# leoelm/Bayesian_inference_for_NN

Measured on AMD Instinct MI355X. Metric: posterior samples/sec (grad-steps/sec) on MLP 784->200->10, batch 1024, higher is better.
Workload: dtype f32; 1 GPU; SGLD, MLP 784->200->10 (D=159010), synthetic MNIST-shaped 48000x784 fp32 resident in HBM, batch 1024 (last batch of an epoch 896), 1 chain per GPU, device-resident run replayed from hipGraphs; seed=2024, parallelism=independent chains x1 (replicas only, no data-path collective)

## Files before the change

### bayesian_inference_for_nn_amd/_build.py

```python

from __future__ import annotations

import fcntl
import glob
import os
import shutil
import subprocess

CSRC = os.path.join(os.path.dirname(os.path.abspath(__file__)), "csrc")
LIB = os.path.join(CSRC, "libpyz.so")
SOURCES = ["pyz_api.hip"]


class NoCompiler(RuntimeError):
    """hipcc is not installed (as opposed to: hipcc ran and failed)."""


def _inputs():
    return ([os.path.join(CSRC, f) for f in SOURCES] + sorted(glob.glob(os.path.join(CSRC, "*.h"))) +
            [os.path.join(CSRC, "..", "..", "include", "pyz.h")])


def _stale() -> bool:
    if not os.path.exists(LIB):
        return True
    t = os.path.getmtime(LIB)
    return any(os.path.exists(p) and os.path.getmtime(p) > t for p in _inputs())


def build(force: bool = False, verbose: bool = False) -> str:
    if not force and not _stale():
        return LIB
    hipcc = shutil.which("hipcc") or "/opt/rocm/bin/hipcc"
    if not os.path.exists(hipcc):
        raise NoCompiler("hipcc not found: cannot build the gfx950 library")
    with open(os.path.join(CSRC, ".build.lock"), "w") as lock:
        fcntl.flock(lock, fcntl.LOCK_EX)
        try:
            if not force and not _stale():
                return LIB
            tmp = LIB + f".tmp{os.getpid()}"
            cmd = [hipcc, "-O3", "-std=c++17", "--offload-arch=gfx950", "-fPIC", "-shared", "-Wall",
                   "-Wno-unused-function", "-Wno-pass-failed"] + SOURCES + ["-o", tmp]
            if verbose:
                print(" ".join(cmd))
            res = subprocess.run(cmd, cwd=CSRC, capture_output=True, text=True)
            if res.returncode != 0:
                if os.path.exists(tmp):
                    os.remove(tmp)
                raise RuntimeError("hipcc failed:\n" + res.stdout + res.stderr)
            os.replace(tmp, LIB)
        finally:
            fcntl.flock(lock, fcntl.LOCK_UN)
    return LIB


if __name__ == "__main__":
    print(build(force=True, verbose=True))
```

### bayesian_inference_for_nn_amd/csrc/pyz_api.hip

```cpp

#include <algorithm>
#include <climits>
#include <cmath>
#include <cstring>
#include <vector>

#include "pyz_common.h"
#include "pyz_corrupt.h"
#include "pyz_fsvi.h"
#include "pyz_fused.h"
#include "pyz_gemm.h"
#include "pyz_gemm_ring.h"
#include "pyz_hmc_fused.h"
#include "pyz_hmc_multi.h"
#include "pyz_input_grad.h"
#include "pyz_pilco.h"
#include "pyz_kernels.h"
#include "pyz_predict_moments.h"
#include "pyz_surface.h"
#include "pyz_rng.h"
#include "pyz_sgld_chains.h"
#include "pyz_sgld_lanes.h"
#include "pyz_members.h"

// ... 4 lines not shown

void drop_graphs(pyz_mlp *m);

int ensure_bytes(void **ptr, size_t *cap, size_t need, pyz_mlp *m) {
  if (*cap >= need) return PYZ_OK;
  if (*ptr) {
    PYZ_HIP(hipDeviceSynchronize());
    PYZ_HIP(hipFree(*ptr));
    drop_graphs(m);
  }
  *ptr = nullptr;
  *cap = 0;
  PYZ_HIP(hipMalloc(ptr, need));
  m->ws_bytes += need;
  *cap = need;
  return PYZ_OK;
}

struct Extra {
  size_t grad_cap = 0, grad2_cap = 0, qsave_cap = 0, part_cap = 0, part2_cap = 0, scal_cap = 0;
  void *hm_buf = nullptr;
  size_t hm_cap = 0;
  void *hm_res_buf = nullptr;
  size_t hm_res_cap = 0;
  void *fwd_part = nullptr;
  size_t fwd_part_cap = 0;
  void *gs_res_buf = nullptr;
  size_t gs_res_cap = 0;
  PyzGraphCache<1> hm_graphs;
  double *part2 = nullptr;
  void *tab_host = nullptr;
  size_t tab_host_cap = 0;
  hipEvent_t tab_ev[2] = {};
  unsigned long long tab_count = 0;
  float2 *tab_bc = nullptr;
  int tab_bc_cap = 0;
  static constexpr int AR_GRAPHS = 32;
  PyzGraphCache<AR_GRAPHS> adam_graphs;
  static constexpr int UP_SLOTS = 64;
  unsigned char *up_host = nullptr;
  size_t up_slot_bytes = 0;
  hipEvent_t up_ev[UP_SLOTS] = {};
  unsigned long long up_count = 0;
  bool hm_fed = false;
  int hm_path = 0;
  unsigned long long hm_sig = 0;
  void *hr_buf = nullptr;
  float *hr_tab = nullptr;
  size_t hr_tab_cap = 0;
  unsigned char *hr_host = nullptr;
  size_t hr_host_cap = 0;
  hipEvent_t hr_ev[2] = {};
  unsigned long long hr_count = 0;
  PyzGraphCache<PYZ_GRAPH_CHUNKS> hmc_run_graphs;
  void *fsvi_buf = nullptr;
  size_t fsvi_cap = 0;
};

}

struct pyz_mlp_full : pyz_mlp {
  Extra x;
};

namespace {

inline pyz_mlp_full *full(pyz_mlp *m) { return static_cast<pyz_mlp_full *>(m); }

void drop_graphs(pyz_mlp *m) {
  m->graphs.drop();
  full(m)->x.hm_graphs.drop();
  full(m)->x.hmc_run_graphs.drop();
  full(m)->x.adam_graphs.drop();
}

int need_grad(pyz_mlp *m, int P) {
  m->grad_owner = 2;
  return ensure_bytes((void **)&m->grad, &full(m)->x.grad_cap, sizeof(float) * (size_t)P * m->D + 64, m);
}
int need_grad2(pyz_mlp *m, int P) {
  return ensure_bytes((void **)&m->grad2, &full(m)->x.grad2_cap, sizeof(float) * (size_t)P * m->D + 64, m);
}
int need_qsave(pyz_mlp *m, int P) {
  return ensure_bytes((void **)&m->qsave, &full(m)->x.qsave_cap, sizeof(float) * (size_t)P * m->D + 64, m);
}
int need_part(pyz_mlp *m, size_t n_doubles) {
  return ensure_bytes((void **)&m->part, &full(m)->x.part_cap, sizeof(double) * n_doubles, m);
}
int need_part2(pyz_mlp *m, size_t n_doubles, bool keep_kernel_matrix = false) {
  if (!keep_kernel_matrix) m->km_valid = false;
  return ensure_bytes((void **)&full(m)->x.part2, &full(m)->x.part2_cap, sizeof(double) * n_doubles, m);
}

int check_call(const pyz_mlp *m, int P, int batch) {
  if (!m) return pyz_fail(PYZ_E_INVALID, "null plan");
  if (batch <= 0 || batch > m->max_batch)
    return pyz_fail(PYZ_E_SHAPE, "batch %d outside [1, %d] of the plan", batch, m->max_batch);
  if (P <= 0 || P > m->max_p)
    return pyz_fail(PYZ_E_SHAPE, "particle count %d outside [1, %d] of the plan", P, m->max_p);
  return PYZ_OK;
}

inline bool aligned16(const void *p) { return (reinterpret_cast<uintptr_t>(p) & 15u) == 0; }

int set_ctl(pyz_mlp *m, int slot, int batch, float lr, long long n, long long row_off, int i, hipStream_t st,
            int slot0 = 0, int n_run = 0) {
  m->pend_on = false;
  PYZ_LAUNCH(k_set_ctl, dim3(1), dim3(1), 0, st, m->ctl + slot, batch, lr, n, row_off, i, slot0, n_run);
  PYZ_LAUNCH_CHECK();
  return PYZ_OK;
}

void set_ctl_lazy(pyz_mlp *m, int batch, float lr, long long n) {
  m->pend = StepCtl{};
  m->pend.batch = batch;
  m->pend.lr = lr;
  m->pend.n = n;
  m->pend_on = true;
}

void flush_ctl(pyz_mlp *m, hipStream_t st) {
  if (!m->pend_on) return;
  m->pend_on = false;
  PYZ_LAUNCH(k_set_ctl, dim3(1), dim3(1), 0, st, m->ctl, m->pend.batch, m->pend.lr, m->pend.n, m->pend.row_off, m->pend.i,
                     m->pend.slot0, 0);
}

DenseArgs forward_args(pyz_mlp *m, int l, const float *theta, long long theta_ps, const float *x, const int32_t *row_idx,
                       const StepCtl *ctl, float *gather_out) {
  DenseArgs g{};
  g.K = m->dims[l];
  g.N = m->dims[l + 1];
  if (l == 0) {
    g.in = x;
    g.in_pstride = 0;
    g.row_idx = row_idx;
    g.gather_out = row_idx ? gather_out : nullptr;
  } else {
    g.in = m->act[l - 1];
    g.in_pstride = (long long)m->max_batch * g.K;
    g.row_idx = nullptr;
  }
  g.lda = g.K;
  g.theta = theta;
  g.theta_pstride = theta_ps;
  g.w_off = m->w_off[l];
  g.out = m->act[l];
  g.out_pstride = (long long)m->max_batch * g.N;
  g.act = m->acts[l];
  g.vec = (g.K % 8 == 0) && aligned16(g.in) ? 1 : 0;
  g.ctl = ctl;
  if (l == 0 && m->pend_on && ctl == m->ctl) {
    g.init = m->pend;
    g.init_on = 1;
    m->pend_on = false;
  }
  return g;
}

void launch_forward(pyz_mlp *m, const float *theta, long long theta_ps, int P, const float *x,
                    const int32_t *row_idx, int grid_batch, const StepCtl *ctl, hipStream_t st,
                    float *gather_out = nullptr, int l_end = -1, const StepCtl *gate = nullptr, int gate_mod = 0) {
  if (l_end < 0) l_end = m->L;
  for (int l = 0; l < l_end; ++l) {
    DenseArgs g = forward_args(m, l, theta, theta_ps, x, row_idx, ctl, gather_out);
    g.wt = pyz_wt_for(P);
    g.gate = gate;
    g.gate_mod = gate_mod;
    if (pyz_launch_fwd_ring(g, grid_batch, P, st)) continue;
    if (!g.row_idx && !g.init_on && !g.gather_out) g.rows_cap = std::min(grid_batch, m->max_batch);
    pyz_launch_fwd(g, grid_batch, P, st);
  }
}

void launch_loss(pyz_mlp *m, int P, const void *y, const int32_t *row_idx, int grid_batch, const StepCtl *ctl,
                 bool want_delta, hipStream_t st) {
  LossArgs g{};
  const int C = m->dims[m->L];
  g.out_last = m->act[m->L - 1];
  g.pstride = (long long)m->max_batch * C;
  g.C = C;
  g.y = y;
  g.delta = want_delta ? m->delta[m->L - 1] : nullptr;
  g.part = m->part;
  g.nblk = cdiv(m->max_batch, 256);
  g.act_last = m->acts[m->L - 1];
  g.ctl = ctl;
  g.row_idx = row_idx;
  dim3 grid(cdiv(grid_batch, 256), P);
  if ((int)grid.x < g.nblk) g.nblk = grid.x;
  if (m->loss == PYZ_LOSS_SCCE)
    PYZ_LAUNCH(k_loss_scce, grid, dim3(256), 0, st, g);
  else
    PYZ_LAUNCH(k_loss_mse, grid, dim3(256), 0, st, g);
}

inline int loss_nblk(const pyz_mlp *m, int grid_batch) { return std::min(cdiv(m->max_batch, 256), cdiv(grid_batch, 256)); }

void launch_backward(pyz_mlp *m, const float *theta, long long theta_ps, int P, const float *x,
                     const int32_t *row_idx, int grid_batch, const StepCtl *ctl, float *grad, hipStream_t st,
                     float *grad_sq = nullptr) {
  for (int l = m->L - 1; l >= 0; --l) {
    const int K = m->dims[l], N = m->dims[l + 1];
    if (l > 0) {
      DenseArgs g{};
      g.K = K;
      g.N = N;
      g.in = m->delta[l];
      g.in_pstride = (long long)m->max_batch * N;
      g.lda = N;
      g.theta = theta;
      g.theta_pstride = theta_ps;
      g.w_off = m->w_off[l];
      g.out = m->delta[l - 1];
      g.out_pstride = (long long)m->max_batch * K;
      g.aux = m->act[l - 1];
      g.aux_pstride = (long long)m->max_batch * K;
      g.act = m->acts[l - 1];
      g.vec = (N % 8 == 0) && (m->w_off[l] % 4 == 0) && (P == 1 || theta_ps % 4 == 0) && aligned16(theta) ? 1 : 0;
      g.ctl = ctl;
      pyz_launch_bwd_data(g, grid_batch, P, st);
    }
    DenseArgs g{};
    g.K = K;
    g.N = N;
    if (l == 0) {
      g.in = x;
      g.in_pstride = 0;
      g.row_idx = row_idx;
    } else {
      g.in = m->act[l - 1];
      g.in_pstride = (long long)m->max_batch * K;
    }
    g.lda = K;
    g.aux = m->delta[l];
    g.aux_pstride = (long long)m->max_batch * N;
    g.out = grad;
    g.out_pstride = m->D;
    g.w_off = m->w_off[l];
    g.ctl = ctl;
    if (grad_sq) pyz_launch_bwd_weight_sq(g, grad_sq, grid_batch, st);
    else pyz_launch_bwd_weight(g, grid_batch, P, st);
  }
}

inline bool can_fuse(const pyz_mlp *m) { return m->dims[m->L] <= 32; }

void launch_head(pyz_mlp *m, const float *theta, long long theta_ps, int P, const float *x, const void *y,
                 const int32_t *row_idx, int grid_batch, const StepCtl *ctl, bool want_delta, hipStream_t st,
                 const StepCtl *gate = nullptr, int gate_mod = 0, int k_split = 0) {
  const int l = m->L - 1;
  HeadArgs g{};
  g.gate = gate;
  g.gate_mod = gate_mod;
  if (k_split > 1) {
    g.hparts = static_cast<const float *>(full(m)->x.fwd_part);
    g.n_hparts = k_split;
    g.hpart_stride = (long long)m->max_batch * m->dims[l];
    g.bias_prev = theta + m->w_off[l - 1] + (long long)m->dims[l - 1] * m->dims[l];
    g.h_store = m->act[l - 1];
  }
  g.K = m->dims[l];
  g.N = m->dims[l + 1];
  if (l == 0) {
    g.hin = x;
    g.hin_pstride = 0;
    g.gather_hin = 1;
  } else {
    g.hin = m->act[l - 1];
    g.hin_pstride = (long long)m->max_batch * g.K;
    g.gather_hin = 0;
  }
  g.lda = g.K;
  g.row_idx = row_idx;
  g.theta = theta;
  g.theta_pstride = theta_ps;
  g.w_off = m->w_off[l];
  g.loss = m->loss;
  g.act_last = m->acts[l];
  g.act_prev = l > 0 ? m->acts[l - 1] : PYZ_ACT_LINEAR;
  g.vec = (g.K % 8 == 0) && aligned16(g.hin) ? 1 : 0;
  g.y = y;
  g.out_last = m->act[l];
  g.delta_last = want_delta ? m->delta[l] : nullptr;
  g.delta_prev = (want_delta && l > 0) ? m->delta[l - 1] : nullptr;
  g.last_pstride = (long long)m->max_batch * g.N;
  g.prev_pstride = (long long)m->max_batch * g.K;
  g.part = m->part;
  g.ctl = ctl;
  g.wt = pyz_wt_for(P);
  if (m->pend_on && ctl == m->ctl) {
    g.init = m->pend;
    g.init_on = 1;
    m->pend_on = false;
  }
  static const int rows_on = pyz_env_int("PYZ_HEAD_ROWS", 1);
  const int UT = g.K <= 64 ? 1 : g.K <= 256 ? 4 : g.K <= 512 ? 8 : g.K <= 1024 ? 16 : 0;
  const int NP = g.N <= 4 ? 4 : g.N <= 8 ? 8 : g.N <= 12 ? 12 : g.N <= 16 ? 16 : g.N <= 24 ? 24 : 32;
  if (rows_on && UT && UT * NP <= 128) {
    g.nblk = grid_batch;
    m->cur_nblk = g.nblk;
    static const int rw_rows = pyz_env_int("PYZ_HEAD_RW_ROWS", 32768);
    const int RW = (long long)P * grid_batch >= rw_rows ? 4 : 1;
    const dim3 grid((unsigned)cdiv(cdiv(grid_batch, RW), 4), P), block(256);
    if (g.n_hparts > 0) {
      if (NP == 4) PYZ_LAUNCH((k_head_rows<4, 4, 1, true>), grid, block, 0, st, g);
      else if (NP == 8) PYZ_LAUNCH((k_head_rows<4, 8, 1, true>), grid, block, 0, st, g);
      else if (NP == 12) PYZ_LAUNCH((k_head_rows<4, 12, 1, true>), grid, block, 0, st, g);
      else PYZ_LAUNCH((k_head_rows<4, 16, 1, true>), grid, block, 0, st, g);
      return;
    }
#define PYZ_HEAD_ROWS_CASE(U, C)                                                               \
  if (UT == U && NP == C) {                                                                    \
    if (RW == 4) PYZ_LAUNCH((k_head_rows<U, C, 4>), grid, block, 0, st, g);                     \
    else PYZ_LAUNCH((k_head_rows<U, C, 1>), grid, block, 0, st, g);                            \
    return;                                                                                    \
  }
    PYZ_HEAD_ROWS_CASE(1, 4) PYZ_HEAD_ROWS_CASE(1, 8) PYZ_HEAD_ROWS_CASE(1, 12) PYZ_HEAD_ROWS_CASE(1, 16)
    PYZ_HEAD_ROWS_CASE(1, 24) PYZ_HEAD_ROWS_CASE(1, 32)
    PYZ_HEAD_ROWS_CASE(4, 4) PYZ_HEAD_ROWS_CASE(4, 8) PYZ_HEAD_ROWS_CASE(4, 12) PYZ_HEAD_ROWS_CASE(4, 16)
    PYZ_HEAD_ROWS_CASE(4, 24) PYZ_HEAD_ROWS_CASE(4, 32)
    PYZ_HEAD_ROWS_CASE(8, 4) PYZ_HEAD_ROWS_CASE(8, 8) PYZ_HEAD_ROWS_CASE(8, 12) PYZ_HEAD_ROWS_CASE(8, 16)
    PYZ_HEAD_ROWS_CASE(16, 4) PYZ_HEAD_ROWS_CASE(16, 8)
#undef PYZ_HEAD_ROWS_CASE
  }
  g.nblk = cdiv(grid_batch, 32);
  m->cur_nblk = g.nblk;
  static const int head_waves = pyz_env_int("PYZ_HEAD_WAVES", 8) >= 8 ? 8 : 4;
  PYZ_LAUNCH(k_head, dim3(g.nblk, P), dim3(64 * head_waves), head_waves * 4096 + 2 * 32 * 33 * 4 + 64, st, g);
}

void launch_bwd_data_hidden(pyz_mlp *m, const float *theta, long long theta_ps, int P, int grid_batch,
                            const StepCtl *ctl, hipStream_t st) {
  for (int l = m->L - 2; l >= 1; --l) {
    const int K = m->dims[l], N = m->dims[l + 1];
    DenseArgs g{};
    g.K = K;
    g.N = N;
    g.in = m->delta[l];
    g.in_pstride = (long long)m->max_batch * N;
    g.lda = N;
    g.theta = theta;
    g.theta_pstride = theta_ps;
    g.w_off = m->w_off[l];
    g.out = m->delta[l - 1];
    g.out_pstride = (long long)m->max_batch * K;
    g.aux = m->act[l - 1];
    g.aux_pstride = (long long)m->max_batch * K;
    g.act = m->acts[l - 1];
    g.vec = (N % 8 == 0) && (m->w_off[l] % 4 == 0) && (P == 1 || theta_ps % 4 == 0) && aligned16(theta) ? 1 : 0;
    g.ctl = ctl;
    pyz_launch_bwd_data(g, grid_batch, P, st);
  }
}

inline int wgrad_tiles(const pyz_mlp *m) {
  int tiles = 0;
  for (int l = 0; l < m->L; ++l) tiles += ((m->dims[l] + 1 + 31) / 32) * ((m->dims[l + 1] + 31) / 32);
  return tiles;
}

int wgrad_layers(pyz_mlp *m, int P, const float *x, const int32_t *row_idx, const StepCtl *ctl, WgradArgs &a,
                 const float *gathered) {
  int tiles = 0;
  a.L = m->L;
  for (int l = 0; l < m->L; ++l) {
    WgradLayer &ly = a.lay[l];
    ly.K = m->dims[l];
    ly.N = m->dims[l + 1];
    if (l == 0) {
      ly.in = (row_idx && gathered) ? gathered : x;
      ly.in_pstride = 0;
      ly.gather = (row_idx && !gathered) ? 1 : 0;
    } else {
      ly.in = m->act[l - 1];
      ly.in_pstride = (long long)m->max_batch * ly.K;
      ly.gather = 0;
    }
    ly.lda = ly.K;
    ly.delta = m->delta[l];
    ly.delta_pstride = (long long)m->max_batch * ly.N;
    ly.w_off = m->w_off[l];
    ly.tile0 = tiles;
    a.tile0[l] = tiles;
    tiles += ((ly.K + 1 + 31) / 32) * ((ly.N + 31) / 32);
  }
  for (int l = m->L; l < PYZ_MAX_LAYERS; ++l) a.tile0[l] = INT_MAX;
  a.row_idx = row_idx;
  a.ctl = ctl;
  a.part = m->part;
  a.nblk = m->cur_nblk;
  a.tiles = tiles;
  a.nonfinite = m->nonfinite;
  a.wt = pyz_wt_for(P);
  return tiles;
}

void launch_wgrad_all(pyz_mlp *m, int P, const float *x, const int32_t *row_idx, int grid_batch, const StepCtl *ctl,
                      WgradArgs &a, hipStream_t st, const float *gathered) {
  const int tiles = wgrad_layers(m, P, x, row_idx, ctl, a, gathered);
  const int S = pyz_pick_waves((long long)tiles * P, (grid_batch + 1) / 2);
  dim3 grid(pyz_pad8((long long)tiles + 1, P), P);
  if (a.prep.src && P == 1) grid.x = (unsigned)(tiles + 1 + std::max(pyz_cu_count() - tiles - 1, 24));
  switch (S) {
    case 1:
      if (a.mode == PYZ_UPD_NONE) PYZ_LAUNCH((k_wgrad_all<1, true>), grid, dim3(64), 0, st, a);
      else PYZ_LAUNCH(k_wgrad_all<1>, grid, dim3(64), 0, st, a);
      break;
    case 2: PYZ_LAUNCH(k_wgrad_all<2>, grid, dim3(128), 2 * 4096, st, a); break;
    case 4: PYZ_LAUNCH(k_wgrad_all<4>, grid, dim3(256), 4 * 4096, st, a); break;
    case 8: PYZ_LAUNCH(k_wgrad_all<8>, grid, dim3(512), 8 * 4096, st, a); break;
    default: PYZ_LAUNCH(k_wgrad_all<16>, grid, dim3(1024), 16 * 4096, st, a); break;
  }
}

void launch_wgrad_adam(pyz_mlp *m, const float *x, const int32_t *row_idx, int grid_batch, const StepCtl *ctl, AdamArgs &a,
                       hipStream_t st, const float *gathered) {
  const int tiles = wgrad_layers(m, 1, x, row_idx, ctl, a.w, gathered);
  const int S = pyz_pick_waves(tiles, (grid_batch + 1) / 2);
  const dim3 grid(tiles + 1);
  switch (S) {
    case 1: PYZ_LAUNCH(k_wgrad_adam<1>, grid, dim3(64), 0, st, a); break;
    case 2: PYZ_LAUNCH(k_wgrad_adam<2>, grid, dim3(128), 2 * 4096, st, a); break;
    case 4: PYZ_LAUNCH(k_wgrad_adam<4>, grid, dim3(256), 4 * 4096, st, a); break;
    case 8: PYZ_LAUNCH(k_wgrad_adam<8>, grid, dim3(512), 8 * 4096, st, a); break;
    default: PYZ_LAUNCH(k_wgrad_adam<16>, grid, dim3(1024), 16 * 4096, st, a); break;
  }
}

void launch_wgrad_bsam(pyz_mlp *m, const float *x, const int32_t *row_idx, int grid_batch, const StepCtl *ctl, int phase,
                       BsamArgs &a, hipStream_t st, const float *gathered) {
  const int tiles = wgrad_layers(m, 1, x, row_idx, ctl, a.w, gathered);
  const int S = pyz_pick_waves(tiles, (grid_batch + 1) / 2);
  const dim3 grid(tiles + 1);
#define PYZ_BSAM_CASE(W, LDS)                                                           \
  if (phase == 0) PYZ_LAUNCH((k_wgrad_bsam<W, 0>), grid, dim3(64 * W), LDS, st, a);     \
  else PYZ_LAUNCH((k_wgrad_bsam<W, 1>), grid, dim3(64 * W), LDS, st, a);                \
  break
  switch (S) {
    case 1: PYZ_BSAM_CASE(1, 0);
    case 2: PYZ_BSAM_CASE(2, 2 * 4096);
    case 4: PYZ_BSAM_CASE(4, 4 * 4096);
    case 8: PYZ_BSAM_CASE(8, 8 * 4096);
    default: PYZ_BSAM_CASE(16, 16 * 4096);
  }
#undef PYZ_BSAM_CASE
}

inline float *batch_buf(pyz_mlp *m, int slot) { return m->xb + (size_t)slot * m->max_batch * m->dims[0]; }

inline bool batch_ahead(const pyz_mlp *m, const int32_t *row_idx) {
  static const int on = pyz_env_int("PYZ_BATCH_AHEAD", 1);
  if (!on || !can_fuse(m) || m->L <= 1 || row_idx == nullptr) return false;
  return on == 2 || wgrad_tiles(m) + 24 <= pyz_cu_count();
}

PrepArgs prep_args(pyz_mlp *m, const float *x, const int32_t *row_idx, int grid_batch, long long row_stride, int dst_slot) {
  PrepArgs p{};
  p.src = x;
  p.dst = batch_buf(m, dst_slot);
  p.row_idx = row_idx;
  p.tab_bs = m->tab_bs;
  p.row_stride = row_stride;
  p.K = p.lda = m->dims[0];
  p.fwd_tiles_n = (m->dims[1] + 31) / 32;
  p.fwd_tiles = ((grid_batch + 31) / 32) * p.fwd_tiles_n;
  return p;
}

int ksplit_for(pyz_mlp *m, const float *theta, long long theta_ps, int P, const float *xc, int grid_batch, const StepCtl *ctl) {
  const int ks_env = pyz_env_int("PYZ_FWD_KSPLIT", 0);
  if (ks_env < 2 || ks_env > 8 || m->L != 2 || P != 1) return 0;
  const int UT = m->dims[1] <= 64 ? 1 : m->dims[1] <= 256 ? 4 : 0, NPc = m->dims[2];
  if (!UT || NPc > 16 || !pyz_env_int("PYZ_HEAD_ROWS", 1)) return 0;
  DenseArgs g = forward_args(m, 0, theta, theta_ps, xc, nullptr, ctl, nullptr);
  if (!pyz_fwd_ring_ksplit_ok(g, grid_batch, P)) return 0;
  if ((long long)((grid_batch + 31) / 32) * ks_env > 2 * pyz_cu_count()) return 0;
  const size_t need = sizeof(float) * (size_t)ks_env * m->max_batch * m->dims[1];
  if (!full(m)->x.fwd_part || full(m)->x.fwd_part_cap < need) return 0;
  return ks_env;
}

void launch_loss_backward(pyz_mlp *m, const float *theta, long long theta_ps, int P, const float *x, const void *y,
                          const int32_t *row_idx, int grid_batch, const StepCtl *ctl, bool want_grad, WgradArgs &upd,
                          hipStream_t st, int ahead_slot = -1, AdamArgs *adam = nullptr) {
  if (can_fuse(m)) {
    if (ahead_slot >= 0) {
      const float *xc = batch_buf(m, ahead_slot);
      const int ks = ksplit_for(m, theta, theta_ps, P, xc, grid_batch, ctl);
      if (ks > 1) {
        DenseArgs g = forward_args(m, 0, theta, theta_ps, xc, nullptr, ctl, nullptr);
        g.wt = pyz_wt_for(P);
        g.k_split = ks;
        g.part_out = static_cast<float *>(full(m)->x.fwd_part);
        g.part_stride = (long long)m->max_batch * g.N;
        pyz_launch_fwd_ring_ksplit(g, grid_batch, st);
      } else {
        launch_forward(m, theta, theta_ps, P, xc, nullptr, grid_batch, ctl, st, nullptr, m->L - 1);
      }
      launch_head(m, theta, theta_ps, P, x, y, row_idx, grid_batch, ctl, want_grad, st, nullptr, 0, ks);
      launch_bwd_data_hidden(m, theta, theta_ps, P, grid_batch, ctl, st);
      launch_wgrad_all(m, P, x, row_idx, grid_batch, ctl, upd, st, xc);
      return;
    }
    static const int use_xb = pyz_env_int("PYZ_GATHER_COPY", 1);
    float *xb = (use_xb && want_grad && row_idx && m->L > 1) ? m->xb : nullptr;
    launch_forward(m, theta, theta_ps, P, x, row_idx, grid_batch, ctl, st, xb, m->L - 1);
    launch_head(m, theta, theta_ps, P, x, y, row_idx, grid_batch, ctl, want_grad, st);
    if (want_grad) {
      launch_bwd_data_hidden(m, theta, theta_ps, P, grid_batch, ctl, st);
      if (adam) launch_wgrad_adam(m, x, row_idx, grid_batch, ctl, *adam, st, xb);
      else launch_wgrad_all(m, P, x, row_idx, grid_batch, ctl, upd, st, xb);
    }
    return;
  }
  flush_ctl(m, st);
  launch_forward(m, theta, theta_ps, P, x, row_idx, grid_batch, ctl, st);
  launch_loss(m, P, y, row_idx, grid_batch, ctl, want_grad, st);
  m->cur_nblk = loss_nblk(m, grid_batch);
  if (want_grad) launch_backward(m, theta, theta_ps, P, x, row_idx, grid_batch, ctl, upd.grad, st, adam ? m->grad2 : nullptr);
}

void launch_bsam_pass(pyz_mlp *m, const float *theta, const float *x, const void *y, const int32_t *row_idx, int grid_batch,
                      int phase, BsamArgs &a, hipStream_t st) {
  static const int use_xb = pyz_env_int("PYZ_GATHER_COPY", 1);
  float *xb = (use_xb && row_idx && m->L > 1) ? m->xb : nullptr;
  launch_forward(m, theta, m->D, 1, x, row_idx, grid_batch, m->ctl, st, xb, m->L - 1);
  launch_head(m, theta, m->D, 1, x, y, row_idx, grid_batch, m->ctl, true, st);
  launch_bwd_data_hidden(m, theta, m->D, 1, grid_batch, m->ctl, st);
  launch_wgrad_bsam(m, x, row_idx, grid_batch, m->ctl, phase, a, st, xb);
}

int check_loss_combo(const pyz_mlp *m) {
  const int last = m->acts[m->L - 1];
  if (m->loss == PYZ_LOSS_SCCE && last != PYZ_ACT_SOFTMAX)
    return pyz_fail(PYZ_E_INVALID, "SparseCategoricalCrossentropy needs a softmax last layer");
  if (m->loss == PYZ_LOSS_MSE && last == PYZ_ACT_SOFTMAX)
    return pyz_fail(PYZ_E_INVALID, "MeanSquaredError on a softmax last layer is not supported");
  if (m->loss == PYZ_LOSS_BCE && (m->dims[m->L] != 1 || last != PYZ_ACT_SIGMOID))
    return pyz_fail(PYZ_E_INVALID, "BinaryCrossentropy needs a last layer of exactly one sigmoid unit");
  return PYZ_OK;
}

AdamScal adam_scalars(float lr, double beta_1, double beta_2, long long epoch, float denom_eps, float decay) {
  AdamScal a;
  a.lr = lr;
  a.b1 = (float)beta_1;
  a.c1 = (float)(1.0 - beta_1);
  a.b2 = (float)beta_2;
  a.c2 = (float)(1.0 - beta_2);
  a.bc1 = (float)(1.0 - std::pow(beta_1, (double)epoch));
  a.bc2 = (float)(1.0 - std::pow(beta_2, (double)epoch));
  a.eps = denom_eps;
  a.decay = decay;
  return a;
}

void launch_delta0(pyz_mlp *m, const float *theta, int P, const float *x, const void *y, int n, hipStream_t st) {
  if (can_fuse(m)) {
    launch_forward(m, theta, m->D, P, x, nullptr, n, m->ctl, st, nullptr, m->L - 1);
    launch_head(m, theta, m->D, P, x, y, nullptr, n, m->ctl, true, st);
    launch_bwd_data_hidden(m, theta, m->D, P, n, m->ctl, st);
    return;
  }
  launch_forward(m, theta, m->D, P, x, nullptr, n, m->ctl, st);
  launch_loss(m, P, y, nullptr, n, m->ctl, true, st);
  m->cur_nblk = loss_nblk(m, n);
  if (m->L > 1) {
    const int l = m->L - 1, K = m->dims[l], N = m->dims[l + 1];
    DenseArgs g{};
    g.K = K;
    g.N = N;
    g.in = m->delta[l];
    g.in_pstride = (long long)m->max_batch * N;
    g.lda = N;
    g.theta = theta;
    g.theta_pstride = m->D;
    g.w_off = m->w_off[l];
    g.out = m->delta[l - 1];
    g.out_pstride = (long long)m->max_batch * K;
    g.aux = m->act[l - 1];
    g.aux_pstride = (long long)m->max_batch * K;
    g.act = m->acts[l - 1];
    g.vec = (N % 8 == 0) && (m->w_off[l] % 4 == 0) && (P == 1 || m->D % 4 == 0) && aligned16(theta) ? 1 : 0;
    g.ctl = m->ctl;
    pyz_launch_bwd_data(g, n, P, st);
  }
  launch_bwd_data_hidden(m, theta, m->D, P, n, m->ctl, st);
}

}

extern "C" {

int pyz_version(void) { return PYZ_VERSION; }

const char *pyz_last_error(void) { return pyz_err_slot().c_str(); }

int pyz_device_count(void) {
  int n = 0;
  if (hipGetDeviceCount(&n) != hipSuccess) return 0;
  return n;
}

int pyz_mlp_create(int n_layers, const int32_t *h_dims, const int32_t *h_acts, int loss, int max_batch,
                   int max_particles, pyz_mlp **out) {
  if (!out || !h_dims || !h_acts) return pyz_fail(PYZ_E_INVALID, "null argument");
  *out = nullptr;
  if (n_layers < 1 || n_layers > PYZ_MAX_LAYERS) return pyz_fail(PYZ_E_INVALID, "n_layers %d outside [1, %d]", n_layers, PYZ_MAX_LAYERS);
  if (max_batch < 1 || max_particles < 1) return pyz_fail(PYZ_E_INVALID, "max_batch and max_particles must be >= 1");
  if (max_particles > 65535) return pyz_fail(PYZ_E_INVALID, "max_particles %d > 65535", max_particles);
  if (loss != PYZ_LOSS_SCCE && loss != PYZ_LOSS_MSE && loss != PYZ_LOSS_BCE) return pyz_fail(PYZ_E_INVALID, "unknown loss %d", loss);
  int ndev = 0;
  if (hipGetDeviceCount(&ndev) != hipSuccess || ndev < 1) return pyz_fail(PYZ_E_NODEV, "no HIP device visible");
  pyz_mlp_full *m = new pyz_mlp_full();
  m->L = n_layers;
  m->loss = loss;
  m->max_batch = max_batch;
  m->max_p = max_particles;
  long long off = 0;
  for (int l = 0; l <= n_layers; ++l) {
    if (h_dims[l] < 1) {
      delete m;
      return pyz_fail(PYZ_E_INVALID, "dims[%d] = %d", l, h_dims[l]);
    }
    m->dims[l] = h_dims[l];
  }
  for (int l = 0; l < n_layers; ++l) {
    const int a = h_acts[l];
    if (a < PYZ_ACT_LINEAR || a > PYZ_ACT_SOFTMAX || (a == PYZ_ACT_SOFTMAX && l != n_layers - 1)) {
      delete m;
      return pyz_fail(PYZ_E_INVALID, "activation %d at layer %d is not supported", a, l);
    }
    m->acts[l] = a;
    m->w_off[l] = off;
    off += (long long)(m->dims[l] + 1) * m->dims[l + 1];
  }
  m->D = off;
  if (loss == PYZ_LOSS_BCE) {
    const int rc = check_loss_combo(m);
    if (rc != PYZ_OK) {
      delete m;
      return rc;
    }
  }
  {
    long long widest = 0;
    for (int l = 0; l <= n_layers; ++l) widest = std::max<long long>(widest, m->dims[l]);
    if ((long long)max_batch * widest * 4 >= (1LL << 31) || off * 4 >= (1LL << 31)) {
      delete m;
      return pyz_fail(PYZ_E_INVALID, "max_batch x widest layer, or the parameter vector, exceeds 2 GiB");
    }
  }
  auto fail = [&](int rc) {
    pyz_mlp_destroy(m);
    return rc;
  };
  for (int l = 0; l < n_layers; ++l) {
    const size_t bytes = sizeof(float) * (size_t)max_particles * max_batch * m->dims[l + 1] + 64;
    if (hipMalloc((void **)&m->act[l], bytes) != hipSuccess || hipMalloc((void **)&m->delta[l], bytes) != hipSuccess)
      return fail(pyz_fail(PYZ_E_OOM, "workspace allocation of %zu bytes failed", bytes));
    m->ws_bytes += 2 * bytes;
  }
  {
    const size_t bytes = 2 * sizeof(float) * (size_t)max_batch * m->dims[0] + 64;
    if (hipMalloc((void **)&m->xb, bytes) != hipSuccess) return fail(pyz_fail(PYZ_E_OOM, "workspace allocation of %zu bytes failed", bytes));
    m->ws_bytes += bytes;
  }
  if (hipMalloc((void **)&m->nonfinite, 64) != hipSuccess || hipMemset(m->nonfinite, 0, 64) != hipSuccess)
    return fail(pyz_fail(PYZ_E_OOM, "counter allocation failed"));
  if (hipMalloc((void **)&m->ctl, 2 * sizeof(StepCtl)) != hipSuccess) return fail(pyz_fail(PYZ_E_OOM, "ctl allocation failed"));
  if (hipMemset(m->ctl, 0, 2 * sizeof(StepCtl)) != hipSuccess) return fail(pyz_fail(PYZ_E_HIP, "ctl memset failed"));
  const size_t scal = sizeof(float) * (size_t)(max_particles * 16 + 64);
  if (hipMalloc((void **)&m->scal, scal) != hipSuccess) return fail(pyz_fail(PYZ_E_OOM, "scalar allocation failed"));
  m->ws_bytes += scal;
  {
    const int rc = need_part(m, (size_t)max_particles * max_batch + 8);
    if (rc != PYZ_OK) return fail(rc);
  }
  if (m->L == 2 && m->dims[1] > 192 && m->dims[1] <= 200 && pyz_env_int("PYZ_FWD_KSPLIT", 0) >= 2) {
    const int rc = ensure_bytes(&m->x.fwd_part, &m->x.fwd_part_cap, sizeof(float) * (size_t)8 * max_batch * m->dims[1], m);
    if (rc != PYZ_OK) return fail(rc);
  }
  {
    const int gs_lds = (int)pyz_svgd_gs_lds_bytes();
    if (hipFuncSetAttribute(reinterpret_cast<const void *>(k_svgd_gs<false>), hipFuncAttributeMaxDynamicSharedMemorySize, gs_lds) != hipSuccess ||
        hipFuncSetAttribute(reinterpret_cast<const void *>(k_svgd_gs<true>), hipFuncAttributeMaxDynamicSharedMemorySize, gs_lds) != hipSuccess)
      return fail(pyz_fail(PYZ_E_HIP, "hipFuncSetAttribute(k_svgd_gs) failed"));
    if (hipFuncSetAttribute(reinterpret_cast<const void *>(k_svgd_gs_resident), hipFuncAttributeMaxDynamicSharedMemorySize,
                            (int)pyz_svgd_gs_res_lds_bytes()) != hipSuccess)
      return fail(pyz_fail(PYZ_E_HIP, "hipFuncSetAttribute(k_svgd_gs_resident) failed"));
    if (hipFuncSetAttribute(reinterpret_cast<const void *>(k_svgd_gs_resident2), hipFuncAttributeMaxDynamicSharedMemorySize,
                            (int)pyz_svgd_gs_res_lds_bytes()) != hipSuccess)
      return fail(pyz_fail(PYZ_E_HIP, "hipFuncSetAttribute(k_svgd_gs_resident2) failed"));
    const int gr_lds = (int)pyz_svgd_gram_lds_bytes();
    if (hipFuncSetAttribute(reinterpret_cast<const void *>(k_svgd_gram_tile<1, false>), hipFuncAttributeMaxDynamicSharedMemorySize, gr_lds) != hipSuccess ||
        hipFuncSetAttribute(reinterpret_cast<const void *>(k_svgd_gram_tile<2, false>), hipFuncAttributeMaxDynamicSharedMemorySize, gr_lds) != hipSuccess ||
        hipFuncSetAttribute(reinterpret_cast<const void *>(k_svgd_gram_tile<4, true>), hipFuncAttributeMaxDynamicSharedMemorySize, gr_lds) != hipSuccess)
      return fail(pyz_fail(PYZ_E_HIP, "hipFuncSetAttribute(k_svgd_gram_tile) failed"));
  }
  *out = m;
  return PYZ_OK;
}

int pyz_mlp_destroy(pyz_mlp *mm) {
  if (!mm) return PYZ_OK;
  pyz_mlp_full *m = full(mm);
  m->graphs.drop();
  m->x.hm_graphs.drop();
  m->x.hmc_run_graphs.drop();
  m->x.adam_graphs.drop();
  for (int l = 0; l < PYZ_MAX_LAYERS; ++l) {
    if (m->act[l]) (void)hipFree(m->act[l]);
    if (m->delta[l]) (void)hipFree(m->delta[l]);
  }
// ... 2777 lines not shown
```

### bayesian_inference_for_nn_amd/csrc/pyz_fused.h

```cpp
#pragma once

#include <type_traits>

#include "pyz_common.h"
#include "pyz_gemm.h"
#include "pyz_kernels.h"

struct HeadArgs {
  const float *hin;
  long long hin_pstride;
  const float *theta;
  long long theta_pstride;
  long long w_off;
  const StepCtl *ctl;
  const int32_t *row_idx;
  const StepCtl *gate;
  const void *y;
  double *part;
  int lda;
  int K, N;
  int loss;
  int gather_hin;
  int gate_mod;
  int init_on;
// ... 112 lines not shown
      const float inv = 1.0f / (float)batch;
#pragma unroll
      for (int q = 0; q < 4; ++q) {
        const int c = lsub + 8 * q;
        if (c < N) {
          const float dv = lvalid ? (expf(zv[q] - lse) - (c == ylab ? 1.0f : 0.0f)) * inv : 0.0f;
          d[c] = dv;
          if (lvalid && dl) dl[c] = dv;
          if (lvalid && ol) ol[c] = zv[q];
        }
      }
    } else if (g.loss == PYZ_LOSS_BCE) {
      if (lsub == 0) {
        const float yv = reinterpret_cast<const float *>(g.y)[yrow];
        float o;
        lm = pyz_bce_row(zv[0], yv, o);
        const float dv = lvalid ? (o - yv) * (1.0f / (float)batch) : 0.0f;
        d[0] = dv;
        if (lvalid && dl) dl[0] = dv;
        if (lvalid && ol) ol[0] = o;
      }
    } else {
      const float *y = reinterpret_cast<const float *>(g.y) + yrow * N;
      const float sc = 2.0f / ((float)batch * (float)N);
      float a = 0.0f;
#pragma unroll
      for (int q = 0; q < 4; ++q) {
        const int c = lsub + 8 * q;
        if (c < N) {
          const float o = pyz_act(zv[q], g.act_last);
          const float e = o - y[c];
          a += e * e;
          const float dv = lvalid ? sc * e * pyz_act_grad(o, g.act_last) : 0.0f;
          d[c] = dv;
          if (lvalid && dl) dl[c] = dv;
          if (lvalid && ol) ol[c] = o;
        }
      }
      lm = pyz_grp8_sum(a) / (float)N;
    }
    const double ws = pyz_wave_sum((lvalid && lsub == 0) ? (double)lm : 0.0);
    if (l == 0) lsum[w] = ws;
  }
  __syncthreads();
  if (threadIdx.x == 0) g.part[p * g.nblk + blockIdx.x] = (lsum[0] + lsum[1]) + (lsum[2] + lsum[3]);
  PYZ_STAMP(1, 4);
  if (!g.delta_prev) return;
  float *op = g.delta_prev + p * g.prev_pstride;
  for (int jt = w; jt < tiles_j; jt += S) {
    const int j0 = jt * 32, jj = j0 + r, j = min(jj, K - 1);
    const float *wp = wl + (long long)j * N;
    float hv[16];
    f32x16 acc = {0};
    if (pre && jt == w) {
#pragma unroll
      for (int i = 0; i < 16; ++i) hv[i] = hv0[i];
#pragma unroll
      for (int q = 0; q < 16; ++q)
        if (q < nsteps) {
          const int kk = 2 * q + h;
          const bool vk = kk < N;
          const float a = vk ? dt[r * 33 + kk] : 0.0f;
          acc = pyz_mfma(a, vk ? bw0[q] : 0.0f, acc);
        }
      PYZ_STAMP(1, 6);
    } else {
#pragma unroll
      for (int i = 0; i < 16; ++i) {
        const int mm = min(m0 + (i & 3) + 8 * (i >> 2) + 4 * h, batch - 1);
        long long row = mm;
        if (g.gather_hin && idx) row = idx[mm];
        hv[i] = hp[row * K + j];
      }
      pyz_steps1_all(
          0, nsteps, acc,
          [&](int s, float &a, float &b) {
            const int kk = 2 * s + h;
            const int kc = kk < N ? kk : 0;
            a = dt[r * 33 + kc];
            b = wp[kc];
          },
          [&](int s, float &a, float &b) {
            const bool vk = 2 * s + h < N;
            a = vk ? a : 0.0f;
            b = vk ? b : 0.0f;
          });
    }
#pragma unroll
    for (int i = 0; i < 16; ++i) {
      const int mm = m0 + (i & 3) + 8 * (i >> 2) + 4 * h;
      if (mm < batch && jj < K) op[(long long)mm * K + jj] = acc[i] * pyz_act_grad(hv[i], g.act_prev);
    }
  }
  PYZ_STAMP(1, 5);
}

__device__ __forceinline__ float pyz_readlane(const float v, const int lane) {
  return __builtin_bit_cast(float, __builtin_amdgcn_readlane(__builtin_bit_cast(int, v), lane));
}
template <int CTRL>
__device__ __forceinline__ float pyz_dpp(const float v) {
  return __builtin_bit_cast(float, __builtin_amdgcn_mov_dpp(__builtin_bit_cast(int, v), CTRL, 0xF, 0xF, true));
}
__device__ __forceinline__ float pyz_row16_allsum(float v) {
  v += pyz_dpp<0xB1>(v);
  v += pyz_dpp<0x4E>(v);
  v += pyz_dpp<0x141>(v);
  v += pyz_dpp<0x140>(v);
  return v;
}

__device__ __forceinline__ float pyz_row16_allmax(float v) {
  v = fmaxf(v, pyz_dpp<0xB1>(v));
  v = fmaxf(v, pyz_dpp<0x4E>(v));
  v = fmaxf(v, pyz_dpp<0x141>(v));
  v = fmaxf(v, pyz_dpp<0x140>(v));
  return v;
}

template <int UT, int NP>
struct PyzHeadW {
  float wv[UT][NP];
  float bias_mine;
};

template <int UT, int NP>
__device__ __forceinline__ void pyz_head_load_w(const HeadArgs &g, const int p, const int l, PyzHeadW<UT, NP> &W) {
  const int K = g.K, N = g.N;
  const float *wl = g.theta + p * g.theta_pstride + g.w_off;
  const __amdgpu_buffer_rsrc_t rw = __builtin_amdgcn_make_buffer_rsrc(const_cast<float *>(wl), 0, (K + 1) * N * 4, 0x00020000);
  constexpr unsigned OOB = 0x7FFFFF00u;
#pragma unroll
  for (int t = 0; t < UT; ++t) {
    const int u = l + 64 * t;
    const unsigned wo = u < K ? 4u * (unsigned)u * (unsigned)N : OOB;
#pragma unroll
    for (int c = 0; c < NP; ++c) W.wv[t][c] = pyz_buf_load(rw, wo + 4u * (unsigned)c, 0u);
  }
  W.bias_mine = pyz_buf_load(rw, l < N ? 4u * ((unsigned)K * (unsigned)N + (unsigned)l) : OOB, 0u);
}

template <int UT>
__device__ __forceinline__ void pyz_head_load_h(const HeadArgs &g, const int p, const long long hrow, const int l, float (&hv)[UT]) {
  const float *hp = g.hin + p * g.hin_pstride + hrow * g.lda;
  const __amdgpu_buffer_rsrc_t rh = __builtin_amdgcn_make_buffer_rsrc(const_cast<float *>(hp), 0, g.K * 4, 0x00020000);
#pragma unroll
  for (int t = 0; t < UT; ++t) hv[t] = pyz_buf_load(rh, 4u * (unsigned)(l + 64 * t), 0u);
}

template <int UT, int NP, bool PRELOADED, bool HP = false>
__device__ __forceinline__ void pyz_head_row(const HeadArgs &g, const int batch, const long long row_off, const int p,
                                             const int m, const int l, PyzHeadW<UT, NP> &W) {
  const int K = g.K, N = g.N;
  int yidx = m;
  if (g.row_idx) yidx = g.row_idx[row_off + m];
  float hv[UT], z[NP];
  if constexpr (HP) {
    const float *pp = g.hparts + (long long)m * K;
    const __amdgpu_buffer_rsrc_t rp = __builtin_amdgcn_make_buffer_rsrc(const_cast<float *>(pp), 0,
        (int)(((long long)(g.n_hparts - 1) * g.hpart_stride + K) * 4), 0x00020000);
    const __amdgpu_buffer_rsrc_t rb = __builtin_amdgcn_make_buffer_rsrc(const_cast<float *>(g.bias_prev), 0, K * 4, 0x00020000);
    constexpr unsigned OOBH = 0x7FFFFF00u;
    float pv[UT][8], bv[UT];
#pragma unroll
    for (int t = 0; t < UT; ++t) {
      const int u = l + 64 * t;
#pragma unroll
      for (int sp = 0; sp < 8; ++sp)
        pv[t][sp] = pyz_buf_load(rp, (u < K && sp < g.n_hparts) ? 4u * (unsigned)(sp * g.hpart_stride + u) : OOBH, 0u);
      bv[t] = pyz_buf_load(rb, 4u * (unsigned)u, 0u);
    }
#pragma unroll
    for (int t = 0; t < UT; ++t) {
      float a = pv[t][0];
#pragma unroll
      for (int sp = 1; sp < 8; ++sp) a += pv[t][sp];
      hv[t] = pyz_act(a + bv[t], g.act_prev);
      const int u = l + 64 * t;
      if (u < K) pyz_st(g.h_store + (long long)m * K + u, hv[t], g.wt);
    }
  } else {
    if (g.gather_hin) {
      asm volatile("; gathered input: the row index is needed here" ::: "memory");
      pyz_head_load_h<UT>(g, p, __builtin_amdgcn_readfirstlane(yidx), l, hv);
    } else {
      pyz_head_load_h<UT>(g, p, m, l, hv);
    }
  }
  if (!PRELOADED) pyz_head_load_w<UT, NP>(g, p, l, W);
  const auto &wv = W.wv;
  const float bias_mine = W.bias_mine;
  asm volatile("; the row index arrives here" : "+v"(yidx));
  const long long yrow = yidx;
  int ylab = 0;
  if (g.loss == PYZ_LOSS_SCCE) ylab = reinterpret_cast<const int32_t *>(g.y)[yrow];
  PYZ_STAMP(1, 1);
#pragma unroll
  for (int c = 0; c < NP; ++c) {
    float a = 0.0f;
#pragma unroll
    for (int t = 0; t < UT; ++t) a = fmaf(hv[t], wv[t][c], a);
    z[c] = a;
  }
#pragma unroll
  for (int c = 0; c < NP; ++c) {
    const float v = pyz_row16_allsum(z[c]);
    z[c] = ((pyz_readlane(v, 0) + pyz_readlane(v, 16)) + (pyz_readlane(v, 32) + pyz_readlane(v, 48))) + pyz_readlane(bias_mine, c);
  }
  PYZ_STAMP(1, 2);
  float d2[NP], lm, my_d = 0.0f, my_o = 0.0f;
  if (g.loss == PYZ_LOSS_SCCE && NP <= 16) {
    const int lc = l & 15;
    float zc = z[0];
#pragma unroll
    for (int c = 1; c < NP; ++c) zc = (lc == c) ? z[c] : zc;
    const bool on = lc < N;
    const float mx = pyz_row16_allmax(on ? zc : -3.0e38f);
    const float exv = on ? expf(zc - mx) : 0.0f;
    const float se = pyz_row16_allsum(exv);
    const float lse = mx + logf(se);
    const bool mine = on && lc == ylab;
    float zy = pyz_row16_allsum(mine ? zc : 0.0f);
    zy = (ylab >= 0 && ylab < N) ? zy : __builtin_nanf("");
    const float inv = 1.0f / (float)batch, rse = 1.0f / se;
    my_d = (exv * rse - (mine ? 1.0f : 0.0f)) * inv;
    my_o = zc;
#pragma unroll
    for (int c = 0; c < NP; ++c) d2[c] = pyz_readlane(my_d, c < 16 ? c : 0);
    lm = lse - zy;
  } else {
    float outv[NP];
    if (g.loss == PYZ_LOSS_SCCE) {
      float mx = -3.0e38f;
#pragma unroll
      for (int c = 0; c < NP; ++c) mx = fmaxf(mx, c < N ? z[c] : -3.0e38f);
      float ex[NP], se = 0.0f;
#pragma unroll
      for (int c = 0; c < NP; ++c) {
        ex[c] = c < N ? expf(z[c] - mx) : 0.0f;
        se += ex[c];
      }
      const float lse = mx + logf(se);
      float zy = __builtin_nanf("");
      const float inv = 1.0f / (float)batch, rse = 1.0f / se;
#pragma unroll
      for (int c = 0; c < NP; ++c) {
        zy = (c == ylab && c < N) ? z[c] : zy;
        d2[c] = (ex[c] * rse - ((c == ylab && c < N) ? 1.0f : 0.0f)) * inv;
        outv[c] = z[c];
      }
      lm = lse - zy;
    } else if (NP == 4 && g.loss == PYZ_LOSS_BCE) {
      const float yv = reinterpret_cast<const float *>(g.y)[yrow];
      float o;
      lm = pyz_bce_row(z[0], yv, o);
      const float dv = (o - yv) * (1.0f / (float)batch);
#pragma unroll
      for (int c = 0; c < NP; ++c) {
        d2[c] = c == 0 ? dv : 0.0f;
        outv[c] = c == 0 ? o : 0.0f;
      }
    } else {
      const float *y = reinterpret_cast<const float *>(g.y) + yrow * N;
      const float sc = 2.0f / ((float)batch * (float)N);
      const int act = g.act_last;
      float a = 0.0f;
#pragma unroll
      for (int c = 0; c < NP; ++c) {
        const float o = pyz_act(z[c], act);
        const float e = o - y[min(c, N - 1)];
        a += c < N ? e * e : 0.0f;
        d2[c] = c < N ? sc * e * pyz_act_grad(o, act) : 0.0f;
        outv[c] = o;
      }
      lm = a / (float)N;
    }
#pragma unroll
    for (int c = 0; c < NP; ++c) {
      my_d = (l == c) ? d2[c] : my_d;
      my_o = (l == c) ? outv[c] : my_o;
    }
  }
  PYZ_STAMP(1, 3);
  if (l < N) {
    if (g.out_last) pyz_st(g.out_last + p * g.last_pstride + (long long)m * N + l, my_o, g.wt);
    if (g.delta_last) pyz_st(g.delta_last + p * g.last_pstride + (long long)m * N + l, my_d, g.wt);
  }
  if (l == 0) g.part[p * g.nblk + m] = (double)lm;
  PYZ_STAMP(1, 4);
  if (!g.delta_prev) return;
  float *op = g.delta_prev + p * g.prev_pstride + (long long)m * K;
  const int actp = g.act_prev;
#pragma unroll
  for (int t = 0; t < UT; ++t) {
    const int u = l + 64 * t;
    float a = 0.0f;
#pragma unroll
    for (int c = 0; c < NP; ++c) a = fmaf(d2[c], wv[t][c], a);
    if (u < K) pyz_st(op + u, a * pyz_act_grad(hv[t], actp), g.wt);
  }
  PYZ_STAMP(1, 5);
}

template <int UT, int NP, int RW = 1, bool HP = false>
__global__ void __launch_bounds__(256) k_head_rows(HeadArgs g) {
  PYZ_STAMP(1, 0);
  const int w = pyz_wave_id(), l = threadIdx.x & 63;
  asm volatile("; arguments in one trip" ::"s"(g.hin), "s"(g.hin_pstride), "s"(g.theta), "s"(g.theta_pstride), "s"(g.w_off),
               "s"(g.ctl), "s"(g.row_idx), "s"(g.gate), "s"(g.y), "s"(g.part), "s"(g.lda), "s"(g.K), "s"(g.N), "s"(g.loss),
               "s"(g.gather_hin), "s"(g.gate_mod), "s"(g.init_on), "s"(g.nblk), "s"(g.act_last), "s"(g.act_prev), "s"(g.vec),
               "s"(g.wt));
  if (g.gate && g.gate->n % g.gate_mod == 0) return;
  StepCtl ctl;
  if (g.init_on) {
    asm volatile("; the step scalars by value" ::: "memory");
    ctl = pyz_ctl_first(g.ctl, g.init, 1);
  } else {
    const PyzCtlHot c = pyz_ctl_arrived(pyz_ctl_request(g.ctl));
    ctl.batch = c.batch;
    ctl.row_off = c.row_off;
  }
  const int batch = ctl.batch, p = blockIdx.y;
  const int m0 = (blockIdx.x * 4 + w) * RW;
  if (m0 >= batch) {
    if (l < RW && m0 + l < g.nblk) g.part[p * g.nblk + m0 + l] = 0.0;
    return;
  }
  PyzHeadW<UT, NP> W;
  if (RW == 1) {
    pyz_head_row<UT, NP, false, HP>(g, batch, ctl.row_off, p, m0, l, W);
    return;
  }
  pyz_head_load_w<UT, NP>(g, p, l, W);
#pragma unroll 1
  for (int rr = 0; rr < RW; ++rr) {
    const int m = m0 + rr;
    if (m >= batch) {
      if (l == 0 && m < g.nblk) g.part[p * g.nblk + m] = 0.0;
      continue;
    }
    pyz_head_row<UT, NP, true>(g, batch, ctl.row_off, p, m, l, W);
  }
}

struct PrepArgs {
  const float *src;
  float *dst;
  const int32_t *row_idx;
  const int32_t *tab_bs;
  long long row_stride;
  int K, lda;
  int fwd_tiles, fwd_tiles_n;
};

__device__ __forceinline__ void pyz_copy_rows(const PrepArgs &g, const int32_t *idx, const int ra, const int rb) {
  const int K = g.K, nt = blockDim.x, t = threadIdx.x;
  if (ra >= rb) return;
  if ((K & 3) == 0 && (g.lda & 3) == 0 && ((reinterpret_cast<uintptr_t>(g.src) | reinterpret_cast<uintptr_t>(g.dst)) & 15) == 0) {
    const int K4 = K >> 2, total = (rb - ra) * K4;
    for (int e0 = t; e0 < total; e0 += 4 * nt) {
      float4 v[4];
#pragma unroll
      for (int u = 0; u < 4; ++u) {
        const int e = min(e0 + u * nt, total - 1), m = ra + e / K4, c = e % K4;
        v[u] = *reinterpret_cast<const float4 *>(g.src + (long long)idx[m] * g.lda + 4 * c);
      }
#pragma unroll
      for (int u = 0; u < 4; ++u) {
        const int e = e0 + u * nt;
        if (e < total) {
          float *d = g.dst + (long long)(ra + e / K4) * K + 4 * (e % K4);
          const f32x4 vv = {v[u].x, v[u].y, v[u].z, v[u].w};
          asm volatile("global_store_dwordx4 %0, %1, off sc1" ::"v"(d), "v"(vv) : "memory");
        }
      }
    }
    return;
  }
  const int total = (rb - ra) * K;
  for (int e = t; e < total; e += nt) {
    const int m = ra + e / K, c = e % K;
    g.dst[(long long)m * K + c] = g.src[(long long)idx[m] * g.lda + c];
  }
}

__device__ __forceinline__ void pyz_prep_rows(const PrepArgs &g, const int32_t *idx, const int nb, const int j, const int cnt,
                                              const int bid) {
  int ra, rb;
  if (cnt >= 8 && g.fwd_tiles >= 8) {
    const int x = bid & 7, q = g.fwd_tiles >> 3, r = g.fwd_tiles & 7;
    const int t0 = x < r ? x * (q + 1) : r * (q + 1) + (x - r) * q, t1 = t0 + (x < r ? q + 1 : q);
    const int b0 = (t0 + g.fwd_tiles_n - 1) / g.fwd_tiles_n, b1 = (t1 + g.fwd_tiles_n - 1) / g.fwd_tiles_n;
    const int r0 = min(32 * b0, nb), r1 = x == 7 ? nb : min(32 * b1, nb);
    const int id0 = bid - j;
    const int first = id0 + ((x - (id0 & 7)) & 7);
    const int mine = (bid - first) >> 3, all = (id0 + cnt - 1 - first) / 8 + 1;
    const int per = (r1 - r0 + all - 1) / all;
    ra = r0 + mine * per;
    rb = min(ra + per, r1);
  } else {
    const int per = (nb + cnt - 1) / cnt;
    ra = j * per;
    rb = min(ra + per, nb);
  }
  pyz_copy_rows(g, idx, ra, rb);
}

__global__ void k_prep_batch(PrepArgs g, const StepCtl *ctl) {
  pyz_prep_rows(g, g.row_idx + ctl->row_off, ctl->batch, (int)blockIdx.x, (int)gridDim.x, (int)blockIdx.x);
}

__global__ void k_run_start(StepCtl *ctl, InlineTabs t, int32_t *tab_bs, float *tab_lr, long long n, long long row_off,
                            int slot0, PrepArgs g) {
  if (blockIdx.x == 0) {
    const int e = threadIdx.x;
    if (e < t.n) {
      tab_bs[e] = t.bs[e];
      tab_lr[e] = t.lr[e];
    }
    if (e == 0) {
      ctl->batch = t.bs[0];
      ctl->lr = t.lr[0];
      ctl->n = n;
      ctl->row_off = row_off;
      ctl->i = 0;
      ctl->slot0 = slot0;
      ctl->n_run = t.n - 1;
    }
  }
  pyz_prep_rows(g, g.row_idx + row_off, t.bs[0], (int)blockIdx.x, (int)gridDim.x, (int)blockIdx.x);
}

__global__ void k_run_start_bc(StepCtl *ctl, InlineTabs t, InlineBc b, int32_t *tab_bs, float *tab_lr, float2 *tab_bc,
                               long long n, long long row_off, int slot0, PrepArgs g) {
  if (blockIdx.x == 0) {
    const int e = threadIdx.x;
    if (e < t.n) {
      tab_bs[e] = t.bs[e];
      tab_lr[e] = t.lr[e];
      tab_bc[e] = b.bc[e];
    }
    if (e == 0) {
      ctl->batch = t.bs[0];
      ctl->lr = t.lr[0];
      ctl->n = n;
      ctl->row_off = row_off;
      ctl->i = 0;
      ctl->slot0 = slot0;
      ctl->n_run = t.n - 1;
    }
  }
  pyz_prep_rows(g, g.row_idx + row_off, t.bs[0], (int)blockIdx.x, (int)gridDim.x, (int)blockIdx.x);
}

struct WgradLayer {
  const float *in;
  long long in_pstride;
  const float *delta;
  long long delta_pstride;
  long long w_off;
  int lda, K, N;
  int tile0;
  int gather;
};

#define PYZ_UPD_NONE 0
#define PYZ_UPD_SGD 1
#define PYZ_UPD_SGLD 2
#define PYZ_UPD_BBB 3
#define PYZ_UPD_SWAG 4

struct WgradArgs {
  int tiles;
  int L;
  int mode;
  int wt;
  const StepCtl *ctl;
  const int32_t *row_idx;
  float *theta, *mean, *sq_mean;
  const float *unit_noise;
  uint64_t seed;
  int tile0[PYZ_MAX_LAYERS];
  const double *part;
  int nblk;
  int loss_indexed;
  float *loss;
  StepCtl *next;
  const int32_t *tab_bs;
  const float *tab_lr;
  int *nonfinite;
  WgradLayer lay[PYZ_MAX_LAYERS];
  float *grad;
  long long grad_pstride;
  float *dev_row;
  int swag_update;
  int swag_freq, swag_k;
  float *dev_base;
  long long dev_stride;
  float alpha, prior_mean, prior_rho, bbb_lr;
  const float *pm_vec, *pr_vec;
  uint32_t bbb_step;
  int bbb_chained;
  const double *part_kl;
  int nblk_kl;
  float *cost;
  float *w_next;
  double *part_kl_next;
  long long row_stride;
  float *ploss;
  PrepArgs prep;
};

static_assert(offsetof(WgradArgs, lay) % 64 == 0 && sizeof(WgradLayer) == 64, "a layer's entry is one 64-byte line");

struct PyzUpdOut {
  float th, mu, sq, dev;
  bool wr_mu, wr_sq, wr_dev;
  float *dev_row;
};

__device__ __forceinline__ PyzUpdOut pyz_update_math(const WgradArgs &g, const int mode, const long long e, const float gv,
                                                     const float th0, const float mu0, const float sq0, const float zz,
                                                     const float lr, const long long nstep) {
  PyzUpdOut o;
  o.th = o.mu = o.sq = o.dev = 0.0f;
  o.wr_mu = o.wr_sq = o.wr_dev = false;
  o.dev_row = nullptr;
  if (mode == PYZ_UPD_SGD) {
    o.th = __builtin_fmaf(-lr, gv, th0);
  } else if (mode == PYZ_UPD_SWAG) {
#pragma clang fp contract(off)
    const float th = __builtin_fmaf(-lr, gv, th0);
    o.th = th;
    const bool upd = g.swag_freq > 0 ? (nstep % g.swag_freq == 0) : (g.swag_update != 0);
    if (upd) {
      const float fn = (float)nstep, fn1 = fn + 1.0f;
      o.mu = (mu0 * fn + th) / fn1;
      o.sq = __builtin_fmaf(th, th, sq0 * fn) / fn1;
      o.dev = th - o.mu;
      o.wr_mu = o.wr_sq = true;
      o.dev_row = g.swag_freq > 0
                      ? g.dev_base + min((nstep + g.swag_freq - 1) / g.swag_freq, (long long)g.swag_k - 1) * g.dev_stride
                      : g.dev_row;
      o.wr_dev = o.dev_row != nullptr;
    }
  } else if (mode == PYZ_UPD_BBB) {
    const float pmean = g.pm_vec ? g.pm_vec[e] : g.prior_mean;
    const float sp = pyz_softplus(g.pr_vec ? g.pr_vec[e] : g.prior_rho), isp2 = 1.0f / (sp * sp);
    const float mu = th0, rho = mu0, wv = sq0;
    const float sg = pyz_softplus(rho), sig = pyz_sigmoid(rho);
    const float d = wv - mu, is2 = 1.0f / (sg * sg);
    const float g_mu = g.alpha * d * is2;
    const float g_rho = g.alpha * (-1.0f / sg + d * d * is2 / sg) * sig;
    const float g_w = gv + g.alpha * (-d * is2 + (wv - pmean) * isp2);
    const float blr = g.bbb_chained ? lr : g.bbb_lr;
    o.th = mu - blr * (g_mu + g_w);
    o.mu = rho - blr * (zz * sig * g_w + g_rho);
    o.wr_mu = true;
  } else if (mode == PYZ_UPD_SGLD) {
#pragma clang fp contract(off)
    const float fn = (float)nstep, fn1 = fn + 1.0f;
    const float gn = __builtin_fmaf(lr, zz, gv);
    const float th = __builtin_fmaf(-lr, gn, th0);
    o.th = th;
    o.mu = (mu0 * fn + th) / fn1;
    o.sq = __builtin_fmaf(th, th, sq0 * fn) / fn1;
    o.wr_mu = o.wr_sq = true;
  }
  return o;
}

__device__ __forceinline__ void pyz_update_store(const WgradArgs &g, const int mode, const long long e, const int p,
                                                 const float gv, const PyzUpdOut &o) {
  if (mode == PYZ_UPD_NONE) {
    g.grad[p * g.grad_pstride + e] = gv;
    return;
  }
  pyz_st(g.theta + e, o.th, g.wt);
  if (o.wr_mu) pyz_st(g.mean + e, o.mu, g.wt);
  if (o.wr_sq) pyz_st(g.sq_mean + e, o.sq, g.wt);
  if (o.wr_dev) o.dev_row[e] = o.dev;
}

__device__ __forceinline__ void pyz_step_duties(const WgradArgs &g, const int l) {
  const int batch = g.ctl->batch;
  if (g.loss) {
    const double v = pyz_sum_partials(g.part, g.nblk);
    if (l == 0) {
      float *lo = g.loss + (g.loss_indexed ? g.ctl->slot0 + g.ctl->i : 0);
      lo[0] = (float)(v / (double)batch);
      pyz_note_loss(g.nonfinite, lo[0]);
      if (g.next) pyz_prepare_next(g.ctl, g.next, g.tab_bs, g.tab_lr, g.row_stride);
    }
  }
  if (g.mode == PYZ_UPD_BBB) {
    const double v = pyz_sum_partials(g.part, g.nblk), k = pyz_sum_partials(g.part_kl, g.nblk_kl);
    if (l == 0) {
      const float loss = (float)(v / (double)batch), kl = (float)k;
      float *co = g.cost + (g.bbb_chained ? 4 * (g.ctl->slot0 + g.ctl->i) : 0);
      co[0] = loss + g.alpha * kl;
      pyz_note_loss(g.nonfinite, co[0]);
      co[1] = loss;
      co[2] = kl;
      if (g.bbb_chained && g.next) pyz_prepare_next(g.ctl, g.next, g.tab_bs, g.tab_lr, g.row_stride);
    }
  }
}


template <class H>
__device__ __forceinline__ void pyz_wgrad_accumulate(f32x16 &acc, const float *abase, const int ic, const float *dbase,
                                                     const int n, const int lda, const int N, const int batch, int s,
                                                     const int se, const int h, const bool is_w, const bool is_b, H hook) {
  const float bconst = is_b ? 1.0f : 0.0f;
  const unsigned a_lane = ((unsigned)h * (unsigned)lda + (unsigned)ic) * 4u;
  const unsigned d_lane = ((unsigned)h * (unsigned)N + (unsigned)n) * 4u;
  const unsigned a_row2 = 8u * (unsigned)lda, d_row2 = 8u * (unsigned)N;
  const __amdgpu_buffer_rsrc_t ra =
      __builtin_amdgcn_make_buffer_rsrc(const_cast<float *>(abase), 0, (int)((unsigned)batch * (unsigned)lda * 4u), 0x00020000);
  const __amdgpu_buffer_rsrc_t rd =
      __builtin_amdgcn_make_buffer_rsrc(const_cast<float *>(dbase), 0, (int)((unsigned)batch * (unsigned)N * 4u), 0x00020000);
  const int full = batch >> 1;
  pyz_steps1_all(
      s, min(se, full), acc,
      [&](int st, float &a, float &d) {
        a = pyz_buf_load(ra, a_lane, (unsigned)PYZ_HOT(st, batch) * a_row2);
        d = pyz_buf_load(rd, d_lane, (unsigned)PYZ_HOT(st, batch) * d_row2);
      },
      [&](int, float &a, float &) { a = is_w ? a : bconst; }, hook);
  if (se > full) {
    const int b = batch - 1;
    float a = abase[(size_t)b * lda + ic], d = dbase[(size_t)b * N + n];
    a = h == 0 ? (is_w ? a : bconst) : 0.0f;
    d = h == 0 ? d : 0.0f;
    acc = pyz_mfma(a, d, acc);
  }
}

template <int S, bool PLAIN, int MODE>
__device__ __forceinline__ void pyz_wgrad_tile(const WgradArgs &g, float *red) {
  constexpr int EPT = 16 / S;
  const int w = pyz_wave_id(), l = threadIdx.x & 63;
  const int r = l & 31, h = l >> 5;
  const int tile = pyz_xcd_remap(blockIdx.x, g.tiles);
  int li = 0;
#pragma unroll
  for (int j = 1; j < PYZ_MAX_LAYERS; ++j) li += tile >= g.tile0[j] ? 1 : 0;
  li = __builtin_amdgcn_readfirstlane(li);
  const WgradLayer &ly = g.lay[li];
  const PyzCtlHot ctl_raw = pyz_ctl_request(g.ctl);
  asm volatile("; the layer in one trip" ::"s"(ly.in), "s"(ly.in_pstride), "s"(ly.delta), "s"(ly.delta_pstride), "s"(ly.w_off),
               "s"(ly.lda), "s"(ly.K), "s"(ly.N), "s"(ly.tile0), "s"(ly.gather));
  const PyzCtlHot ctl = pyz_ctl_arrived(ctl_raw);
  const int batch = ctl.batch;
  const int K = ly.K, N = ly.N;
  const int tiles_n = (N + 31) >> 5;
  const int t = tile - ly.tile0;
  const int i0 = (t / tiles_n) * 32, n0 = (t % tiles_n) * 32;
  const int p = blockIdx.y;
  const long long w_off = ly.w_off;
  constexpr int mode = PLAIN ? PYZ_UPD_NONE : MODE;
  const long long nstep = ctl.n;
  const float lr = ctl.lr;

  long long ee[EPT];
  bool ev[EPT];
  float th0[PLAIN ? 1 : EPT], mu0[PLAIN ? 1 : EPT], sq0[PLAIN ? 1 : EPT], zz[PLAIN ? 1 : EPT];
  float zg[PLAIN ? 1 : EPT];
  float zn[PLAIN ? 1 : EPT];
  const bool fuse_next = !PLAIN && mode == PYZ_UPD_BBB && g.w_next != nullptr;
  auto prefetch = [&]() {
#pragma unroll
    for (int q = 0; q < EPT; ++q) {
      int ro, co;
      if (S == 1) {
        ro = (q & 3) + 8 * (q >> 2) + 4 * h;
        co = r;
      } else {
        const int e = threadIdx.x + q * 64 * S;
        ro = e >> 5;
        co = e & 31;
      }
      const int ii = i0 + ro, nn = n0 + co;
      ev[q] = ii <= K && nn < N;
      ee[q] = w_off + (long long)min(ii, K) * N + min(nn, N - 1);
      if (PLAIN) continue;
      th0[q] = mu0[q] = sq0[q] = zz[q] = zg[q] = 0.0f;
      if (mode != PYZ_UPD_NONE) th0[q] = g.theta[ee[q]];
      if (mode == PYZ_UPD_SGLD || mode == PYZ_UPD_BBB || mode == PYZ_UPD_SWAG) {
        mu0[q] = g.mean[ee[q]];
        sq0[q] = g.sq_mean[ee[q]];
        if (g.unit_noise && mode != PYZ_UPD_SWAG) zz[q] = g.unit_noise[ee[q]];
      }
    }
    if (!PLAIN && (mode == PYZ_UPD_SGLD || mode == PYZ_UPD_BBB) && !g.unit_noise) {
#pragma unroll
      for (int q = 0; q < EPT; ++q) {
        zg[q] = mode == PYZ_UPD_SGLD ? pyz_normal1(g.seed, PYZ_STREAM_SGLD, (uint32_t)nstep, (uint64_t)ee[q])
                                     : pyz_normal1(g.seed, PYZ_STREAM_BBB, g.bbb_chained ? (uint32_t)nstep : g.bbb_step, (uint64_t)ee[q]);
      }
    }
    if (!PLAIN && fuse_next) {
#pragma unroll
      for (int q = 0; q < EPT; ++q) zn[q] = pyz_normal1(g.seed, PYZ_STREAM_BBB, (uint32_t)(nstep + 1), (uint64_t)ee[q]);
    }
  };

  const int i = i0 + r, n = min(n0 + r, N - 1);
  const int ic = min(i, K - 1);
  const bool is_w = i < K, is_b = i == K;
  const float *ap = ly.in + p * ly.in_pstride + ic;
  const float *dp = ly.delta + p * ly.delta_pstride + n;
  const int32_t *idx = (ly.gather && g.row_idx) ? g.row_idx + ctl.row_off : nullptr;
  f32x16 acc = {0};
  const int steps = (batch + 1) >> 1;
  int s = (steps * w) / S;
  const int se = (steps * (w + 1)) / S;
  PYZ_STAMP(2, 1);
  if (idx) {
    prefetch();
    for (int s0 = s; s0 < se; s0 += 32) {
      const int idxv = idx[min(2 * s0 + l, batch - 1)];
      const int lda = ly.lda;
      pyz_steps1_all(
          s0, min(s0 + 32, se), acc,
          [&](int st, float &a, float &d) {
            const int bc = PYZ_HOT(min(2 * st + h, batch - 1), batch);
            const long long row = PYZ_HOT(__shfl(idxv, 2 * (st - s0) + h, 64), batch);
            a = ap[row * lda];
            d = dp[(long long)bc * N];
          },
          [&](int st, float &a, float &d) {
            const bool vb = 2 * st + h < batch;
            a = vb ? (is_w ? a : (is_b ? 1.0f : 0.0f)) : 0.0f;
            d = vb ? d : 0.0f;
          });
    }
  } else {
    pyz_wgrad_accumulate(acc, ly.in + p * ly.in_pstride, ic, ly.delta + p * ly.delta_pstride, n, ly.lda, N, batch, s, se, h,
                         is_w, is_b, prefetch);
  }
  PYZ_STAMP(2, 2);
  float gv[EPT];
  if (S == 1) {
#pragma unroll
    for (int q = 0; q < EPT; ++q) gv[q] = acc[q];
  } else {
    float *my = red + w * 1024;
#pragma unroll
    for (int q = 0; q < 16; ++q) my[((q & 3) + 8 * (q >> 2) + 4 * h) * 32 + r] = acc[q];
    __syncthreads();
#pragma unroll
    for (int q = 0; q < EPT; ++q) {
      const int e = threadIdx.x + q * 64 * S;
      float v = red[e];
#pragma unroll
      for (int ww = 1; ww < S; ++ww) v += red[ww * 1024 + e];
      gv[q] = v;
    }
  }
  PYZ_STAMP(2, 4);
  double klp = 0.0;
  float sp_s = 1.0f, lsp_s = 0.0f;
  if (!PLAIN && fuse_next) {
    sp_s = pyz_softplus(g.prior_rho);
    lsp_s = logf(sp_s);
  }
#pragma unroll
  for (int q = 0; q < EPT; ++q) {
    if (!ev[q]) continue;
    if (PLAIN) {
      pyz_st(g.grad + p * g.grad_pstride + ee[q], gv[q], g.wt);
      continue;
    }
    const PyzUpdOut o = pyz_update_math(g, mode, ee[q], gv[q], th0[q], mu0[q], sq0[q],
                                        PLAIN ? 0.0f : (g.unit_noise ? zz[q] : zg[q]), lr, nstep);
    pyz_update_store(g, mode, ee[q], p, gv[q], o);
    if (fuse_next) {
      const long long e = ee[q];
      const float pmean = g.pm_vec ? g.pm_vec[e] : g.prior_mean;
      float sp = sp_s, lsp = lsp_s;
      if (g.pr_vec) {
        sp = pyz_softplus(g.pr_vec[e]);
        lsp = logf(sp);
      }
      const float mu = o.th, sg = pyz_softplus(o.mu);
      const float wn = zn[q] * sg + mu;
      pyz_st(g.w_next + e, wn, g.wt);
      const float a = (wn - mu) / sg, b = (wn - pmean) / sp;
      const float lq = -0.5f * a * a - logf(sg) - PYZ_LOG_SQRT_2PI;
      const float lp = -0.5f * b * b - lsp - PYZ_LOG_SQRT_2PI;
      klp += (double)lq - (double)lp;
    }
  }
  if (!PLAIN && fuse_next) {
    double tot = pyz_wave_sum(klp);
    if (S > 1) {
      double *sm = reinterpret_cast<double *>(red);
      __syncthreads();
      if (l == 0) sm[w] = tot;
      __syncthreads();
      tot = 0.0;
      if (threadIdx.x == 0)
        for (int ww = 0; ww < S; ++ww) tot += sm[ww];
    }
    if (threadIdx.x == 0) g.part_kl_next[blockIdx.x] = tot;
  }
  PYZ_STAMP(2, 3);
}

template <int S, bool PLAIN = false>
__global__ void __launch_bounds__(64 * S) k_wgrad_all(WgradArgs g) {
  extern __shared__ float red[];
  PYZ_STAMP(2, 0);
  const int w = pyz_wave_id(), l = threadIdx.x & 63;
  asm volatile("; arguments in one trip" ::"s"(g.tiles), "s"(g.mode), "s"(g.ctl), "s"(g.row_idx), "s"(g.tile0[1]),
               "s"(g.tile0[2]), "s"(g.tile0[3]), "s"(g.tile0[4]), "s"(g.tile0[5]), "s"(g.tile0[6]), "s"(g.tile0[7]),
               "s"(g.tile0[8]), "s"(g.tile0[9]), "s"(g.tile0[10]), "s"(g.tile0[11]), "s"(g.tile0[12]), "s"(g.tile0[13]),
               "s"(g.tile0[14]), "s"(g.tile0[15]));
  if (blockIdx.x >= (unsigned)g.tiles) {
    if (blockIdx.x == (unsigned)g.tiles && blockIdx.y == 0 && w == 0) pyz_step_duties(g, l);
    if (blockIdx.x == (unsigned)g.tiles && w == 0 && g.ploss) {
      const double tot = pyz_sum_partials(g.part + (long long)blockIdx.y * g.nblk, g.nblk);
      if (l == 0) {
        g.ploss[blockIdx.y] = (float)(tot / (double)g.ctl->batch);
        pyz_note_loss(g.nonfinite, g.ploss[blockIdx.y]);
      }
    }
    if (!PLAIN && blockIdx.x > (unsigned)g.tiles && blockIdx.y == 0 && g.prep.src) {
      const int i2 = g.ctl->i + 1;
      if (i2 < g.ctl->n_run)
        pyz_prep_rows(g.prep, g.prep.row_idx + g.ctl->row_off + g.prep.row_stride, g.prep.tab_bs[i2],
                      (int)blockIdx.x - g.tiles - 1, (int)gridDim.x - g.tiles - 1, (int)blockIdx.x);
      PYZ_STAMP(2, 3);
    }
    return;
  }
  if constexpr (PLAIN) {
    pyz_wgrad_tile<S, true, PYZ_UPD_NONE>(g, red);
  } else {
    switch (g.mode) {
      case PYZ_UPD_SGLD: pyz_wgrad_tile<S, false, PYZ_UPD_SGLD>(g, red); break;
      case PYZ_UPD_SGD: pyz_wgrad_tile<S, false, PYZ_UPD_SGD>(g, red); break;
      case PYZ_UPD_SWAG: pyz_wgrad_tile<S, false, PYZ_UPD_SWAG>(g, red); break;
      case PYZ_UPD_BBB: pyz_wgrad_tile<S, false, PYZ_UPD_BBB>(g, red); break;
      default: pyz_wgrad_tile<S, false, PYZ_UPD_NONE>(g, red); break;
    }
  }
}

template <class H>
__device__ __forceinline__ void pyz_wgrad_accumulate_sq(f32x16 &acc, f32x16 &acc2, const float fb, const float *abase,
                                                        const int ic, const float *dbase, const int n, const int lda,
                                                        const int N, const int batch, int s, const int se, const int h,
                                                        const bool is_w, const bool is_b, H hook) {
  const float bconst = is_b ? 1.0f : 0.0f;
  const unsigned a_lane = ((unsigned)h * (unsigned)lda + (unsigned)ic) * 4u;
  const unsigned d_lane = ((unsigned)h * (unsigned)N + (unsigned)n) * 4u;
  const unsigned a_row2 = 8u * (unsigned)lda, d_row2 = 8u * (unsigned)N;
  const __amdgpu_buffer_rsrc_t ra =
      __builtin_amdgcn_make_buffer_rsrc(const_cast<float *>(abase), 0, (int)((unsigned)batch * (unsigned)lda * 4u), 0x00020000);
  const __amdgpu_buffer_rsrc_t rd =
      __builtin_amdgcn_make_buffer_rsrc(const_cast<float *>(dbase), 0, (int)((unsigned)batch * (unsigned)N * 4u), 0x00020000);
  const int full = batch >> 1;
  pyz_steps1_all(
      s, min(se, full), acc,
      [&](int st, float &a, float &d) {
        a = pyz_buf_load(ra, a_lane, (unsigned)PYZ_HOT(st, batch) * a_row2);
        d = pyz_buf_load(rd, d_lane, (unsigned)PYZ_HOT(st, batch) * d_row2);
      },
      [&](int, float &a, float &d) {
        a = is_w ? a : bconst;
        const float gd = d * fb;
        acc2 = pyz_mfma(a * a, gd * gd, acc2);
      },
      hook);
  if (se > full) {
    const int b = batch - 1;
    float a = abase[(size_t)b * lda + ic], d = dbase[(size_t)b * N + n];
    a = h == 0 ? (is_w ? a : bconst) : 0.0f;
    d = h == 0 ? d : 0.0f;
    const float gd = d * fb;
    acc2 = pyz_mfma(a * a, gd * gd, acc2);
    acc = pyz_mfma(a, d, acc);
  }
}

struct AdamArgs {
  WgradArgs w;
  float *m, *v;
  AdamScal a;
};

struct RunChain {
  const float2 *tab_bc;
  int perturb;
  float lam, num_data;
};

__device__ __forceinline__ void pyz_run_duties(const WgradArgs &g, const int l, const int stride, const int off,
                                               const bool advance) {
  const double v = pyz_sum_partials(g.part, g.nblk);
  if (l == 0) {
    float *lo = g.loss + (long long)stride * (g.ctl->slot0 + g.ctl->i) + off;
    lo[0] = (float)(v / (double)g.ctl->batch);
    pyz_note_loss(g.nonfinite, lo[0]);
    if (advance) pyz_prepare_next(g.ctl, g.next, g.tab_bs, g.tab_lr, g.row_stride);
  }
}

__device__ __forceinline__ void pyz_run_prep(const WgradArgs &g) {
  if (blockIdx.x > (unsigned)g.tiles && g.prep.src) {
    const int i2 = g.ctl->i + 1;
    if (i2 < g.ctl->n_run)
      pyz_prep_rows(g.prep, g.prep.row_idx + g.ctl->row_off + g.prep.row_stride, g.prep.tab_bs[i2],
                    (int)blockIdx.x - g.tiles - 1, (int)gridDim.x - g.tiles - 1, (int)blockIdx.x);
  }
}

struct AdamRunArgs : AdamArgs {
  RunChain c;
};

template <int S, bool CHAIN = false>
__global__ void __launch_bounds__(64 * S) k_wgrad_adam(std::conditional_t<CHAIN, AdamRunArgs, AdamArgs> A) {
  extern __shared__ float red[];
  const WgradArgs &g = A.w;
  constexpr int EPT = 16 / S;
  const int w = pyz_wave_id(), l = threadIdx.x & 63;
  const int r = l & 31, h = l >> 5;
  if (blockIdx.x >= (unsigned)g.tiles) {
    if constexpr (CHAIN) {
      if (blockIdx.x == (unsigned)g.tiles && w == 0) pyz_run_duties(g, l, 1, 0, true);
      pyz_run_prep(g);
    } else {
      if (blockIdx.x == (unsigned)g.tiles && w == 0) pyz_step_duties(g, l);
    }
    return;
  }
  const int tile = pyz_xcd_remap(blockIdx.x, g.tiles);
  int li = 0;
  while (li + 1 < g.L && tile >= g.lay[li + 1].tile0) ++li;
  const WgradLayer &ly = g.lay[li];
  const int batch = g.ctl->batch;
  const int K = ly.K, N = ly.N;
  const int tiles_n = (N + 31) >> 5;
  const int t = tile - ly.tile0;
  const int i0 = (t / tiles_n) * 32, n0 = (t % tiles_n) * 32;
  const long long w_off = ly.w_off;

  long long ee[EPT];
  bool ev[EPT];
  float th0[EPT], m0[EPT], v0[EPT];
  float zn[CHAIN ? EPT : 1];
  AdamScal sc;
  bool perturb_next = false;
  if constexpr (CHAIN) {
    const int si = g.ctl->i;
    const float2 bc = A.c.tab_bc[si];
    sc = A.a;
    sc.lr = g.ctl->lr;
    sc.bc1 = bc.x;
    sc.bc2 = bc.y;
    perturb_next = A.c.perturb && si + 1 < g.ctl->n_run;
  }
  auto prefetch = [&]() {
#pragma unroll
    for (int q = 0; q < EPT; ++q) {
      int ro, co;
      if (S == 1) {
        ro = (q & 3) + 8 * (q >> 2) + 4 * h;
        co = r;
      } else {
        const int e = threadIdx.x + q * 64 * S;
        ro = e >> 5;
        co = e & 31;
      }
      const int ii = i0 + ro, nn = n0 + co;
      ev[q] = ii <= K && nn < N;
      ee[q] = w_off + (long long)min(ii, K) * N + min(nn, N - 1);
      th0[q] = g.theta[ee[q]];
      m0[q] = A.m[ee[q]];
      v0[q] = A.v[ee[q]];
    }
    if constexpr (CHAIN) {
      if (perturb_next) {
        const uint32_t n1 = (uint32_t)(g.ctl->n + 1);
#pragma unroll
        for (int q = 0; q < EPT; ++q) zn[q] = pyz_normal1(g.seed, PYZ_STREAM_VADAM, n1, (uint64_t)ee[q]);
      }
    }
  };

  const int i = i0 + r, n = min(n0 + r, N - 1);
  const int ic = min(i, K - 1);
  const bool is_w = i < K, is_b = i == K;
  const float *ap = ly.in + ic;
  const float *dp = ly.delta + n;
  const int32_t *idx = (ly.gather && g.row_idx) ? g.row_idx + g.ctl->row_off : nullptr;
  const float fb = (float)batch;
  f32x16 acc = {0}, acc2 = {0};
  const int steps = (batch + 1) >> 1;
  int s = (steps * w) / S;
  const int se = (steps * (w + 1)) / S;
  if (idx) {
    prefetch();
    for (int s0 = s; s0 < se; s0 += 32) {
      const int idxv = idx[min(2 * s0 + l, batch - 1)];
      const int lda = ly.lda;
      pyz_steps1_all(
          s0, min(s0 + 32, se), acc,
          [&](int st, float &a, float &d) {
            const int bc = min(2 * st + h, batch - 1);
            const long long row = __shfl(idxv, 2 * (st - s0) + h, 64);
            a = ap[row * lda];
            d = dp[(long long)bc * N];
          },
          [&](int st, float &a, float &d) {
            const bool vb = 2 * st + h < batch;
            a = vb ? (is_w ? a : (is_b ? 1.0f : 0.0f)) : 0.0f;
            d = vb ? d : 0.0f;
            const float gd = d * fb;
            acc2 = pyz_mfma(a * a, gd * gd, acc2);
          });
    }
  } else {
    pyz_wgrad_accumulate_sq(acc, acc2, fb, ly.in, ic, ly.delta, n, ly.lda, N, batch, s, se, h, is_w, is_b, prefetch);
  }
  float gv[EPT], sv[EPT];
  if (S == 1) {
#pragma unroll
    for (int q = 0; q < EPT; ++q) {
      gv[q] = acc[q];
      sv[q] = acc2[q];
    }
  } else {
    float *my = red + w * 1024;
#pragma unroll
    for (int q = 0; q < 16; ++q) my[((q & 3) + 8 * (q >> 2) + 4 * h) * 32 + r] = acc[q];
    __syncthreads();
#pragma unroll
    for (int q = 0; q < EPT; ++q) {
      const int e = threadIdx.x + q * 64 * S;
      float v = red[e];
#pragma unroll
      for (int ww = 1; ww < S; ++ww) v += red[ww * 1024 + e];
      gv[q] = v;
    }
    __syncthreads();
#pragma unroll
    for (int q = 0; q < 16; ++q) my[((q & 3) + 8 * (q >> 2) + 4 * h) * 32 + r] = acc2[q];
    __syncthreads();
#pragma unroll
    for (int q = 0; q < EPT; ++q) {
      const int e = threadIdx.x + q * 64 * S;
      float v = red[e];
#pragma unroll
      for (int ww = 1; ww < S; ++ww) v += red[ww * 1024 + e];
      sv[q] = v;
    }
  }
#pragma unroll
  for (int q = 0; q < EPT; ++q) {
    if (!ev[q]) continue;
    if constexpr (CHAIN) {
      const PyzAdamOut o = pyz_adam_math_pinned(sc, th0[q], m0[q], v0[q], gv[q], sv[q] / fb);
      const float th = perturb_next ? pyz_vadam_perturb_math(A.c.num_data, A.c.lam, o.th, o.v, zn[q]) : o.th;
      pyz_st(g.theta + ee[q], th, g.wt);
      pyz_st(A.m + ee[q], o.m, g.wt);
      pyz_st(A.v + ee[q], o.v, g.wt);
    } else {
      const PyzAdamOut o = pyz_adam_math(A.a, th0[q], m0[q], v0[q], gv[q], sv[q] / fb);
      pyz_st(g.theta + ee[q], o.th, g.wt);
      pyz_st(A.m + ee[q], o.m, g.wt);
      pyz_st(A.v + ee[q], o.v, g.wt);
    }
  }
}


struct BsamArgs {
  WgradArgs w;
  float *m, *v, *g1;
  BsamScal a;
};

struct BsamRunArgs : BsamArgs {
  RunChain c;
};

template <int S, int PHASE, bool CHAIN = false>
__global__ void __launch_bounds__(64 * S) k_wgrad_bsam(std::conditional_t<CHAIN, BsamRunArgs, BsamArgs> A) {
  extern __shared__ float red[];
  const WgradArgs &g = A.w;
  constexpr int EPT = 16 / S;
  const int w = pyz_wave_id(), l = threadIdx.x & 63;
  const int r = l & 31, h = l >> 5;
  if (blockIdx.x >= (unsigned)g.tiles) {
    if constexpr (CHAIN) {
      if (blockIdx.x == (unsigned)g.tiles && w == 0) pyz_run_duties(g, l, 2, PHASE, PHASE == 1);
      if constexpr (PHASE == 1) pyz_run_prep(g);
    } else {
      if (blockIdx.x == (unsigned)g.tiles && w == 0) pyz_step_duties(g, l);
    }
    return;
  }
  const int tile = pyz_xcd_remap(blockIdx.x, g.tiles);
  int li = 0;
  while (li + 1 < g.L && tile >= g.lay[li + 1].tile0) ++li;
  const WgradLayer &ly = g.lay[li];
  const int batch = g.ctl->batch;
  const int K = ly.K, N = ly.N;
  const int tiles_n = (N + 31) >> 5;
  const int t = tile - ly.tile0;
  const int i0 = (t / tiles_n) * 32, n0 = (t % tiles_n) * 32;
  const long long w_off = ly.w_off;

  long long ee[EPT];
  bool ev[EPT];
  float th0[EPT], v0[EPT], m0[PHASE ? EPT : 1], g10[PHASE ? EPT : 1];
  float zn[(CHAIN && PHASE) ? EPT : 1];
  BsamScal sc;
  bool perturb_next = false;
  if constexpr (CHAIN) {
    sc = A.a;
    sc.lr = g.ctl->lr;
    if constexpr (PHASE == 1) perturb_next = A.c.perturb && g.ctl->i + 1 < g.ctl->n_run;
  }
  auto prefetch = [&]() {
#pragma unroll
    for (int q = 0; q < EPT; ++q) {
      int ro, co;
      if (S == 1) {
        ro = (q & 3) + 8 * (q >> 2) + 4 * h;
        co = r;
      } else {
        const int e = threadIdx.x + q * 64 * S;
        ro = e >> 5;
        co = e & 31;
      }
      const int ii = i0 + ro, nn = n0 + co;
      ev[q] = ii <= K && nn < N;
      ee[q] = w_off + (long long)min(ii, K) * N + min(nn, N - 1);
      th0[q] = g.theta[ee[q]];
      v0[q] = A.v[ee[q]];
      if constexpr (PHASE == 1) {
        m0[q] = A.m[ee[q]];
        g10[q] = A.g1[ee[q]];
      }
    }
    if constexpr (CHAIN && PHASE == 1) {
      if (perturb_next) {
// ... 78 lines not shown
```

### bayesian_inference_for_nn_amd/csrc/pyz_gemm.h

```cpp
#pragma once

#include <cstdlib>

#include "pyz_common.h"

struct DenseArgs {
  const float *in;
  long long in_pstride;
  const float *theta;
  long long theta_pstride;
  long long w_off;
  int lda;
  int K, N;
  int vec;
  int rows_cap;
  int gate_mod;
  float *out;
  long long out_pstride;
  const StepCtl *ctl;
  const int32_t *row_idx;
  float *gather_out;
  const StepCtl *gate;
  int act;
  int wt;
  int init_on;
  const float *aux;
  long long aux_pstride;
  StepCtl init;
  int n_part, grid_rows;
  int n_cgrp, cgrp_w;
  int k_split;
  float *part_out;
  long long part_stride;
};

__device__ __forceinline__ int pyz_xcd_remap(const int bid, const int n) {
  const int q = n >> 3, r = n & 7, x = bid & 7, local = bid >> 3;
  return (x < r ? x * (q + 1) : r * (q + 1) + (x - r) * q) + local;
}

#ifdef PYZ_EXP_HOT
#define PYZ_HOT(v, batch) ((v) & ((batch) < 0 ? -1 : 0))
#else
#define PYZ_HOT(v, batch) (v)
#endif

__device__ __forceinline__ f32x16 pyz_mfma(float a, float b, f32x16 c) {
#ifdef PYZ_EXP_NOMFMA
  c[0] += a * b;
  return c;
#else
  return __builtin_amdgcn_mfma_f32_32x32x2f32(a, b, c, 0, 0, 0);
#endif
}

__device__ __forceinline__ float pyz_act(float z, int act) {
  switch (act) {
    case PYZ_ACT_RELU: return z < 0.0f ? 0.0f : z;
    case PYZ_ACT_TANH: return tanhf(z);
    case PYZ_ACT_SIGMOID: return 1.0f / (1.0f + expf(-z));
    default: return z;
  }
}

__device__ __forceinline__ float pyz_act_grad(float h, int act) {
  switch (act) {
    case PYZ_ACT_RELU: return h > 0.0f ? 1.0f : 0.0f;
    case PYZ_ACT_TANH: return 1.0f - h * h;
    case PYZ_ACT_SIGMOID: return h * (1.0f - h);
    default: return 1.0f;
  }
}

__device__ __forceinline__ float pyz_bce_row(float z, float y, float &p) {
  const float e = expf(-fabsf(z));
  const float r = 1.0f / (1.0f + e);
  p = z >= 0.0f ? r : (z < 0.0f ? e * r : z);
  const float u = 1.0f + e;
  const float l1p = u == 1.0f ? e : logf(u) * (e / (u - 1.0f));
  return fmaxf(z, 0.0f) - z * y + l1p;
}

template <int S, class F>
__device__ __forceinline__ void pyz_tile_combine(const float *red, F &store) {
  constexpr int EPT = 16 / S;
  float v[EPT][S];
#pragma unroll
  for (int q = 0; q < EPT; ++q)
#pragma unroll
    for (int ww = 0; ww < S; ++ww) v[q][ww] = red[ww * 1024 + (int)threadIdx.x + q * 64 * S];
#pragma unroll
  for (int q = 0; q < EPT; ++q) {
    const int e = (int)threadIdx.x + q * 64 * S;
    float s = v[q][0];
#pragma unroll
    for (int ww = 1; ww < S; ++ww) s += v[q][ww];
    store(e >> 5, e & 31, s);
  }
}

template <class F>
__device__ __forceinline__ void pyz_tile_epilogue(const f32x16 &acc, float *red, F store) {
  const int S = blockDim.x >> 6, w = pyz_wave_id(), l = threadIdx.x & 63;
  const int r = l & 31, h = l >> 5;
  if (S == 1) {
#pragma unroll
    for (int i = 0; i < 16; ++i) store((i & 3) + 8 * (i >> 2) + 4 * h, r, acc[i]);
    return;
  }
  float *my = red + w * 1024;
#pragma unroll
  for (int i = 0; i < 16; ++i) my[((i & 3) + 8 * (i >> 2) + 4 * h) * 32 + r] = acc[i];
  __syncthreads();
  switch (S) {
    case 2: pyz_tile_combine<2>(red, store); break;
    case 4: pyz_tile_combine<4>(red, store); break;
    case 8: pyz_tile_combine<8>(red, store); break;
    case 16: pyz_tile_combine<16>(red, store); break;
    default: __builtin_trap();
  }
}

struct PyzNoFix {
  __device__ __forceinline__ void operator()(int, float &, float &) const {}
};

struct PyzNoHook {
  __device__ __forceinline__ void operator()() const {}
};

template <int G, class L, class F, class H = PyzNoHook>
__device__ __forceinline__ void pyz_pipe1(int s, const int se, f32x16 &acc, L load, F fix, H hook = H()) {
  if (s >= se) {
    hook();
    return;
  }
  float an[G], bn[G], a[G], b[G];
  const int last = se - 1;
#pragma unroll
  for (int u = 0; u < G; ++u) load(min(s + u, last), an[u], bn[u]);
  __builtin_amdgcn_sched_barrier(0);
  hook();
  __builtin_amdgcn_sched_barrier(0);
  for (;;) {
#pragma unroll
    for (int u = 0; u < G; ++u) {
      a[u] = an[u];
      b[u] = bn[u];
    }
    const int sn = s + G;
    if (sn < se) {
#pragma unroll
      for (int u = 0; u < G; ++u) load(min(sn + u, last), an[u], bn[u]);
    }
    __builtin_amdgcn_sched_barrier(0);
#pragma unroll
    for (int u = 0; u < G; ++u)
      if (s + u < se) {
        fix(s + u, a[u], b[u]);
        acc = pyz_mfma(a[u], b[u], acc);
      }
    __builtin_amdgcn_sched_barrier(0);
    s = sn;
    if (s >= se) break;
  }
}

#define PYZ_MFMA4(A, B)              \
  acc = pyz_mfma((A).x, (B).x, acc); \
  acc = pyz_mfma((A).y, (B).y, acc); \
  acc = pyz_mfma((A).z, (B).z, acc); \
  acc = pyz_mfma((A).w, (B).w, acc);

struct PyzNoUse4 {
  __device__ __forceinline__ void operator()(int, const float4 &) const {}
};

template <int G, class L, class U, class H = PyzNoHook>
__device__ __forceinline__ void pyz_pipe4(int c, const int ce, f32x16 &acc, L load, U use, H hook = H()) {
  if (c >= ce) {
    hook();
    return;
  }
  float4 an[G], bn[G], a[G], b[G];
  const int last = ce - 1;
#pragma unroll
  for (int u = 0; u < G; ++u) load(min(c + u, last), an[u], bn[u]);
  __builtin_amdgcn_sched_barrier(0);
  hook();
  __builtin_amdgcn_sched_barrier(0);
  for (;;) {
#pragma unroll
    for (int u = 0; u < G; ++u) {
      a[u] = an[u];
      b[u] = bn[u];
    }
    const int cn = c + G;
    if (cn < ce) {
#pragma unroll
      for (int u = 0; u < G; ++u) load(min(cn + u, last), an[u], bn[u]);
    }
    __builtin_amdgcn_sched_barrier(0);
#pragma unroll
    for (int u = 0; u < G; ++u)
      if (c + u < ce) {
        use(c + u, a[u]);
        PYZ_MFMA4(a[u], b[u])
      }
    __builtin_amdgcn_sched_barrier(0);
    c = cn;
    if (c >= ce) break;
  }
}

template <class L, class U, class H = PyzNoHook>
__device__ __forceinline__ void pyz_steps4_all(int c, const int ce, f32x16 &acc, L load, U use, H hook = H()) {
  pyz_pipe4<2>(c, ce, acc, load, use, hook);
}
template <class L, class F, class H = PyzNoHook>
__device__ __forceinline__ void pyz_steps1_all(int s, const int se, f32x16 &acc, L load, F fix, H hook = H()) {
  pyz_pipe1<8>(s, se, acc, load, fix, hook);
}

__device__ __forceinline__ float pyz_buf_load(const __amdgpu_buffer_rsrc_t rsrc, const unsigned voff, const unsigned soff) {
  return __builtin_bit_cast(float, __builtin_amdgcn_raw_buffer_load_b32(rsrc, (int)voff, (int)soff, 0));
}

template <class H = PyzNoHook>
__device__ __forceinline__ void pyz_fwd_accumulate(f32x16 &acc, const float *ap, const float *wl, const int n, const int K,
                                                   const int N, const int vec, const int w, const int S, const int h,
                                                   float *gp = nullptr, const int copy_mod = 1, const int copy_rem = 0,
                                                   H hook = H()) {
  const __amdgpu_buffer_rsrc_t rw =
      __builtin_amdgcn_make_buffer_rsrc(const_cast<float *>(wl), 0, (int)((unsigned)(K + 1) * (unsigned)N * 4u), 0x00020000);
  const unsigned n4 = 4u * (unsigned)n, N4 = 4u * (unsigned)N;
  const float bias = pyz_buf_load(rw, n4, (unsigned)K * N4);
  const int c8 = vec ? (K >> 3) : 0;
  const unsigned v0 = (4u * h) * N4 + n4, v1 = v0 + N4, v2 = v1 + N4, v3 = v2 + N4;
  pyz_steps4_all(
      0, (c8 - w + S - 1) / S, acc,
      [&](int u, float4 &a4, float4 &b4) {
        const int c = PYZ_HOT(w + S * u, K);
        a4 = *reinterpret_cast<const float4 *>(ap + 8 * c + 4 * h);
        const unsigned so = 8u * (unsigned)c * N4;
        b4 = make_float4(pyz_buf_load(rw, v0, so), pyz_buf_load(rw, v1, so), pyz_buf_load(rw, v2, so), pyz_buf_load(rw, v3, so));
      },
      [&](int u, const float4 &a4) {
        const int c = w + S * u;
        if (gp && c % copy_mod == copy_rem) {
#ifdef PYZ_COPY_NT
          typedef float pyz_f4 __attribute__((ext_vector_type(4)));
          pyz_f4 v = {a4.x, a4.y, a4.z, a4.w};
          __builtin_nontemporal_store(v, reinterpret_cast<pyz_f4 *>(gp + 8 * c + 4 * h));
#else
          *reinterpret_cast<float4 *>(gp + 8 * c + 4 * h) = a4;
#endif
        }
      },
      hook);
  const int t0 = 8 * c8, steps = (K - t0 + 1) >> 1;
  const unsigned vt = (unsigned)h * N4 + n4;
  pyz_steps1_all(
      0, (steps - w + S - 1) / S, acc,
      [&](int u, float &a, float &b) {
        const int kb = t0 + 2 * (w + S * u);
        const int kk = kb + h;
        a = ap[kk < K ? kk : 0];
        b = pyz_buf_load(rw, vt, (unsigned)kb * N4);
      },
      [&](int u, float &a, float &b) {
        const int kk = t0 + 2 * (w + S * u) + h;
        const bool vk = kk < K;
        if (gp && vk && copy_rem == 0) gp[kk] = a;
        a = vk ? a : 0.0f;
        b = vk ? b : 0.0f;
      });
  if (w == 0) {
    acc = pyz_mfma(h == 0 ? 1.0f : 0.0f, h == 0 ? bias : 0.0f, acc);
  }
}

__global__ void k_dense_fwd(DenseArgs g) {
  extern __shared__ float red[];
  PYZ_STAMP(0, 0);
  const int S = blockDim.x >> 6, w = pyz_wave_id(), l = threadIdx.x & 63;
  const int r = l & 31, h = l >> 5;
  const int tiles_n = (g.N + 31) >> 5;
  asm volatile("; arguments in one trip" ::"s"(g.in), "s"(g.in_pstride), "s"(g.theta), "s"(g.theta_pstride), "s"(g.w_off),
               "s"(g.lda), "s"(g.K), "s"(g.N), "s"(g.vec), "s"(g.rows_cap), "s"(g.gate_mod), "s"(g.out), "s"(g.out_pstride),
               "s"(g.ctl), "s"(g.row_idx), "s"(g.gather_out), "s"(g.gate), "s"(g.act), "s"(g.wt), "s"((int)gridDim.x),
               "s"((int)blockDim.x));
  if (g.gate && g.gate->n % g.gate_mod == 0) return;
  const int tile = pyz_xcd_remap(blockIdx.x, gridDim.x);
  const int m0 = (tile / tiles_n) * 32, n0 = (tile % tiles_n) * 32;
  int cap = g.rows_cap;
  long long row_off = 0;
  if (cap <= 0) {
    asm volatile("; the step scalars are needed here" ::: "memory");
    const StepCtl ctl = pyz_ctl_first(g.ctl, g.init, g.init_on);
    cap = __builtin_amdgcn_readfirstlane(ctl.batch);
    row_off = ctl.row_off;
  }
  if (m0 >= cap) return;
  const int p = blockIdx.y;
  const int K = g.K, N = g.N;
  const int m = min(m0 + r, cap - 1), n = min(n0 + r, N - 1);
  long long row = m;
  if (g.row_idx) row = g.row_idx[row_off + m];
  const float *ap = g.in + p * g.in_pstride + row * g.lda;
  const float *wl = g.theta + p * g.theta_pstride + g.w_off;
  f32x16 acc = {0};
  PYZ_STAMP(0, 1);
  float *gp = (g.gather_out && p == 0) ? g.gather_out + (long long)m * K : nullptr;
  int batch = 0;
  const int32_t *ctl_batch = &g.ctl->batch;
  pyz_fwd_accumulate(acc, ap, wl, n, K, N, g.vec, w, S, h, gp, tiles_n, tile % tiles_n,
                     [&]() { batch = __hip_atomic_load(ctl_batch, __ATOMIC_RELAXED, __HIP_MEMORY_SCOPE_AGENT); });
  batch = g.rows_cap > 0 ? __builtin_amdgcn_readfirstlane(batch) : cap;
  PYZ_STAMP(0, 2);
  float *op = g.out + p * g.out_pstride;
  const int act = g.act, wt = g.wt;
  pyz_tile_epilogue(acc, red, [&](int ro, int co, float v) {
    const int mm = m0 + ro, nn = n0 + co;
    if (mm < batch && nn < N) pyz_st(op + (long long)mm * N + nn, pyz_act(v, act), wt);
  });
  PYZ_STAMP(0, 3);
}

template <int NT>
__global__ void __launch_bounds__(256) k_dense_fwd_lds(DenseArgs g) {
  constexpr int BN = 32 * NT, BM = 128, BK = 16;
  constexpr int AS = BM + 32;
  constexpr int BS = (BN % 64 == 0) ? BN + 32 : BN;
  constexpr int BJ = NT;
  __shared__ __attribute__((aligned(16))) float As[2][BK][AS];
  __shared__ __attribute__((aligned(16))) float Bs[2][BK][BS];
  const int t = threadIdx.x, w = pyz_wave_id(), l = t & 63, r = l & 31, h = l >> 5;
  const StepCtl ctl = pyz_ctl_first(g.ctl, g.init, g.init_on);
  const int batch = ctl.batch;
  const int K = g.K, N = g.N;
  const int tiles_n = (N + BN - 1) / BN;
  const int tile = pyz_xcd_remap(blockIdx.x, gridDim.x);
  const int m0 = (tile / tiles_n) * BM, n0 = (tile % tiles_n) * BN;
  if (m0 >= batch) return;
  const int p = blockIdx.y;
  const int ra = t >> 1, ka = 8 * (t & 1);
  const int ma = min(m0 + ra, batch - 1);
  long long rowa = ma;
  if (g.row_idx) rowa = g.row_idx[ctl.row_off + ma];
  const float *ap = g.in + p * g.in_pstride + rowa * g.lda + ka;
  const float *wl = g.theta + p * g.theta_pstride + g.w_off;
  float *gp = (g.gather_out && p == 0 && n0 == 0 && m0 + ra < batch) ? g.gather_out + (long long)ma * K + ka : nullptr;
  float4 va[2];
  float2 vb[BJ];
  auto fetch = [&](const int k0) {
#pragma unroll
    for (int j = 0; j < 2; ++j) {
      const int k = k0 + ka + 4 * j;
      va[j] = k < K ? *reinterpret_cast<const float4 *>(ap + k0 + 4 * j) : make_float4(0.f, 0.f, 0.f, 0.f);
    }
#pragma unroll
    for (int j = 0; j < BJ; ++j) {
      const int idx = t + 256 * j, kr = idx / (BN / 2), c2 = idx % (BN / 2);
      const int k = k0 + kr, n = n0 + 2 * c2;
      vb[j] = (k < K && n < N) ? *reinterpret_cast<const float2 *>(wl + (long long)k * N + n) : make_float2(0.f, 0.f);
    }
  };
  auto stage = [&](const int buf, const int k0) {
#pragma unroll
    for (int j = 0; j < 2; ++j) {
      const int kk = ka + 4 * j;
      As[buf][kk + 0][ra] = va[j].x;
      As[buf][kk + 1][ra] = va[j].y;
      As[buf][kk + 2][ra] = va[j].z;
      As[buf][kk + 3][ra] = va[j].w;
      if (gp && k0 + kk < K) *reinterpret_cast<float4 *>(gp + k0 + 4 * j) = va[j];
    }
#pragma unroll
    for (int j = 0; j < BJ; ++j) {
      const int idx = t + 256 * j, kr = idx / (BN / 2), c2 = idx % (BN / 2);
      *reinterpret_cast<float2 *>(&Bs[buf][kr][2 * c2]) = vb[j];
    }
  };
  f32x16 acc[NT];
#pragma unroll
  for (int nt = 0; nt < NT; ++nt) acc[nt] = f32x16{0};
  const int ns = (K + BK - 1) / BK;
  PYZ_STAMP(0, 0);
  fetch(0);
  stage(0, 0);
  __syncthreads();
  PYZ_STAMP(0, 1);
  for (int s = 0; s < ns; ++s) {
    const int buf = s & 1;
    if (s == 24) PYZ_STAMP(0, 2);
    if (s + 1 < ns) fetch((s + 1) * BK);
#pragma unroll
    for (int kp = 0; kp < BK / 2; ++kp) {
      const float a = As[buf][2 * kp + h][32 * w + r];
#pragma unroll
      for (int nt = 0; nt < NT; ++nt) acc[nt] = pyz_mfma(a, Bs[buf][2 * kp + h][32 * nt + r], acc[nt]);
    }
    if (s == 24) PYZ_STAMP(0, 3);
    if (s + 1 < ns) stage(buf ^ 1, (s + 1) * BK);
    if (s == 24) PYZ_STAMP(0, 4);
    __syncthreads();
    if (s == 24) PYZ_STAMP(0, 5);
  }
  PYZ_STAMP(0, 6);
  float *op = g.out + p * g.out_pstride;
  const int act = g.act, wt = g.wt;
  const bool wide = (N & 3) == 0 && (g.out_pstride & 3) == 0 && (reinterpret_cast<uintptr_t>(g.out) & 15) == 0;
  if (wide) {
    __syncthreads();
    float *tw = &As[0][0][0] + 1024 * w;
    static_assert(2 * BK * AS >= 4 * 1024, "tile scratch");
    const int tr = l >> 3, tc = 4 * (l & 7);
#pragma unroll
    for (int nt = 0; nt < NT; ++nt) {
      const int nn = n0 + 32 * nt + r;
      const float bias = nn < N ? wl[(long long)K * N + nn] : 0.0f;
#pragma unroll
      for (int i = 0; i < 16; ++i) tw[((i & 3) + 8 * (i >> 2) + 4 * h) * 32 + r] = pyz_act(acc[nt][i] + bias, act);
#pragma unroll
      for (int q = 0; q < 4; ++q) {
        const int ro = tr + 8 * q, mm = m0 + 32 * w + ro, nc = n0 + 32 * nt + tc;
        const float4 v = *reinterpret_cast<const float4 *>(tw + ro * 32 + tc);
        if (mm < batch && nc < N) {
          float *d = op + (long long)mm * N + nc;
          if (wt) {
            const f32x4 vv = {v.x, v.y, v.z, v.w};
            asm volatile("global_store_dwordx4 %0, %1, off sc1" ::"v"(d), "v"(vv) : "memory");
          } else {
            *reinterpret_cast<float4 *>(d) = v;
          }
        }
      }
    }
    PYZ_STAMP(0, 7);
    return;
  }
#pragma unroll
  for (int nt = 0; nt < NT; ++nt) {
    const int nn = n0 + 32 * nt + r;
    if (nn < N) {
      const float bias = wl[(long long)K * N + nn];
#pragma unroll
      for (int i = 0; i < 16; ++i) {
        const int mm = m0 + 32 * w + (i & 3) + 8 * (i >> 2) + 4 * h;
        if (mm < batch) pyz_st(op + (long long)mm * N + nn, pyz_act(acc[nt][i] + bias, act), wt);
      }
    }
  }
  PYZ_STAMP(0, 7);
}

__global__ void k_dense_bwd_data(DenseArgs g) {
  extern __shared__ float red[];
  const int S = blockDim.x >> 6, w = pyz_wave_id(), l = threadIdx.x & 63;
  const int r = l & 31, h = l >> 5;
  const int batch = g.ctl->batch;
  const int K = g.K, N = g.N;
  const int tiles_j = (K + 31) >> 5;
  const int tile = pyz_xcd_remap(blockIdx.x, gridDim.x);
  const int m0 = (tile / tiles_j) * 32, j0 = (tile % tiles_j) * 32;
  if (m0 >= batch) return;
  const int p = blockIdx.y;
  const int m = min(m0 + r, batch - 1), j = min(j0 + r, K - 1);
  const float *ap = g.in + p * g.in_pstride + (long long)m * N;
  const float *wp = g.theta + p * g.theta_pstride + g.w_off + (long long)j * N;
  f32x16 acc = {0};
  const int c8 = g.vec ? (N >> 3) : 0;
  pyz_steps4_all(
      (c8 * w) / S, (c8 * (w + 1)) / S, acc,
      [&](int c, float4 &a4, float4 &b4) {
        const int k = 8 * c + 4 * h;
        a4 = *reinterpret_cast<const float4 *>(ap + k);
        b4 = *reinterpret_cast<const float4 *>(wp + k);
      },
      PyzNoUse4());
  {
    const int t0 = 8 * c8, steps = (N - t0 + 1) >> 1;
    pyz_steps1_all(
        (steps * w) / S, (steps * (w + 1)) / S, acc,
        [&](int s, float &a, float &b) {
          const int kk = t0 + 2 * s + h;
          const int kc = kk < N ? kk : 0;
          a = ap[kc];
          b = wp[kc];
        },
        [&](int s, float &a, float &b) {
          const bool vk = t0 + 2 * s + h < N;
          a = vk ? a : 0.0f;
          b = vk ? b : 0.0f;
        });
  }
  float *op = g.out + p * g.out_pstride;
  const float *hp = g.aux + p * g.aux_pstride;
  const int act = g.act, wt = g.wt;
  pyz_tile_epilogue(acc, red, [&](int ro, int co, float v) {
    const int mm = m0 + ro, jj = j0 + co;
    if (mm < batch && jj < K) {
      const long long o = (long long)mm * K + jj;
      pyz_st(op + o, v * pyz_act_grad(hp[o], act), wt);
    }
  });
}

template <int G, bool GATHER, bool SQ = false>
__device__ __forceinline__ void pyz_wgrad_steps(int &s, const int se, f32x16 &acc, const float *ap, const float *dp,
                                                const int32_t *idx, const int lda, const int N, const int batch,
                                                const int h, const int r, const bool is_w, const bool is_b,
                                                f32x16 *acc2 = nullptr, const float dsc = 0.0f) {
  for (; s + G <= se; s += G) {
    float a[G], d[G];
    int idxv = 0;
    if (GATHER) idxv = idx[min(2 * s + r, batch - 1)];
#pragma unroll
    for (int u = 0; u < G; ++u) {
      const int b = 2 * (s + u) + h;
      const bool vb = b < batch;
      const int bc = vb ? b : 0;
      long long row = bc;
      if (GATHER) row = __shfl(idxv, 2 * u + h, 64);
      const float av = ap[row * lda], dv = dp[(long long)bc * N];
      a[u] = av;
      d[u] = dv;
    }
    __builtin_amdgcn_sched_barrier(0);
#pragma unroll
    for (int u = 0; u < G; ++u) {
      const bool vb = 2 * (s + u) + h < batch;
      const float av = vb ? (is_w ? a[u] : (is_b ? 1.0f : 0.0f)) : 0.0f;
      acc = pyz_mfma(av, vb ? d[u] : 0.0f, acc);
      if constexpr (SQ) {
        const float gd = (vb ? d[u] : 0.0f) * dsc;
        *acc2 = pyz_mfma(av * av, gd * gd, *acc2);
      }
    }
    __builtin_amdgcn_sched_barrier(0);
  }
}

__global__ void k_dense_bwd_weight(DenseArgs g) {
  extern __shared__ float red[];
  const int S = blockDim.x >> 6, w = pyz_wave_id(), l = threadIdx.x & 63;
  const int r = l & 31, h = l >> 5;
  const int batch = g.ctl->batch;
  const int K = g.K, N = g.N;
  const int tiles_n = (N + 31) >> 5;
  const int tile = pyz_xcd_remap(blockIdx.x, gridDim.x);
  const int i0 = (tile / tiles_n) * 32, n0 = (tile % tiles_n) * 32;
  const int p = blockIdx.y;
  const int i = i0 + r, n = min(n0 + r, N - 1);
  const int ic = min(i, K - 1);
  const bool is_w = i < K, is_b = i == K;
  const float *ap = g.in + p * g.in_pstride + ic;
  const float *dp = g.aux + p * g.aux_pstride + n;
  const int32_t *idx = g.row_idx ? g.row_idx + g.ctl->row_off : nullptr;
  f32x16 acc = {0};
  const int steps = (batch + 1) >> 1;
  int s = (steps * w) / S;
  const int se = (steps * (w + 1)) / S;
  if (idx) {
    pyz_wgrad_steps<16, true>(s, se, acc, ap, dp, idx, g.lda, N, batch, h, r, is_w, is_b);
    pyz_wgrad_steps<4, true>(s, se, acc, ap, dp, idx, g.lda, N, batch, h, r, is_w, is_b);
    pyz_wgrad_steps<1, true>(s, se, acc, ap, dp, idx, g.lda, N, batch, h, r, is_w, is_b);
  } else {
    pyz_wgrad_steps<16, false>(s, se, acc, ap, dp, idx, g.lda, N, batch, h, r, is_w, is_b);
    pyz_wgrad_steps<4, false>(s, se, acc, ap, dp, idx, g.lda, N, batch, h, r, is_w, is_b);
    pyz_wgrad_steps<1, false>(s, se, acc, ap, dp, idx, g.lda, N, batch, h, r, is_w, is_b);
  }
  float *op = g.out + p * g.out_pstride + g.w_off;
  pyz_tile_epilogue(acc, red, [&](int ro, int co, float v) {
    const int ii = i0 + ro, nn = n0 + co;
    if (ii <= K && nn < N) op[(long long)ii * N + nn] = v;
  });
}

__global__ void k_dense_bwd_weight_sq(DenseArgs g, float *out2) {
  extern __shared__ float red[];
  const int S = blockDim.x >> 6, w = pyz_wave_id(), l = threadIdx.x & 63;
  const int r = l & 31, h = l >> 5;
  const int batch = g.ctl->batch;
  const int K = g.K, N = g.N;
  const int tiles_n = (N + 31) >> 5;
  const int tile = pyz_xcd_remap(blockIdx.x, gridDim.x);
  const int i0 = (tile / tiles_n) * 32, n0 = (tile % tiles_n) * 32;
  const int i = i0 + r, n = min(n0 + r, N - 1);
  const int ic = min(i, K - 1);
  const bool is_w = i < K, is_b = i == K;
  const float *ap = g.in + ic;
  const float *dp = g.aux + n;
  const int32_t *idx = g.row_idx ? g.row_idx + g.ctl->row_off : nullptr;
  const float fb = (float)batch;
  f32x16 acc = {0}, acc2 = {0};
  const int steps = (batch + 1) >> 1;
  int s = (steps * w) / S;
  const int se = (steps * (w + 1)) / S;
  if (idx) {
    pyz_wgrad_steps<16, true, true>(s, se, acc, ap, dp, idx, g.lda, N, batch, h, r, is_w, is_b, &acc2, fb);
    pyz_wgrad_steps<4, true, true>(s, se, acc, ap, dp, idx, g.lda, N, batch, h, r, is_w, is_b, &acc2, fb);
    pyz_wgrad_steps<1, true, true>(s, se, acc, ap, dp, idx, g.lda, N, batch, h, r, is_w, is_b, &acc2, fb);
  } else {
    pyz_wgrad_steps<16, false, true>(s, se, acc, ap, dp, idx, g.lda, N, batch, h, r, is_w, is_b, &acc2, fb);
    pyz_wgrad_steps<4, false, true>(s, se, acc, ap, dp, idx, g.lda, N, batch, h, r, is_w, is_b, &acc2, fb);
    pyz_wgrad_steps<1, false, true>(s, se, acc, ap, dp, idx, g.lda, N, batch, h, r, is_w, is_b, &acc2, fb);
  }
  float *op = g.out + g.w_off, *op2 = out2 + g.w_off;
  pyz_tile_epilogue(acc, red, [&](int ro, int co, float v) {
    const int ii = i0 + ro, nn = n0 + co;
    if (ii <= K && nn < N) op[(long long)ii * N + nn] = v;
  });
  __syncthreads();
  pyz_tile_epilogue(acc2, red, [&](int ro, int co, float v) {
    const int ii = i0 + ro, nn = n0 + co;
    if (ii <= K && nn < N) op2[(long long)ii * N + nn] = v / fb;
  });
}

static inline int pyz_env_int(const char *name, int dflt) {
  const char *v = getenv(name);
  return v && *v ? atoi(v) : dflt;
}

static inline int pyz_cu_count() {
  static const int n = [] {
    int dev = 0, v = 0;
    if (hipGetDevice(&dev) != hipSuccess || hipDeviceGetAttribute(&v, hipDeviceAttributeMultiprocessorCount, dev) != hipSuccess || v <= 0)
      v = 256;
    return v;
  }();
  return n;
}

static inline int pyz_wt_for(int P) {
  static const int on = pyz_env_int("PYZ_WT", 1);
  return (on == 2 || (on && P == 1)) ? 1 : 0;
}

static inline int pyz_pick_waves(long long tiles, long long mfma_steps) {
  static const int target = pyz_env_int("PYZ_WAVES_TARGET", 3072);
  static const int min_steps = pyz_env_int("PYZ_MIN_STEPS", 8);
  int S = 1;
  while (S < 16 && tiles * S < target && mfma_steps / (2 * S) >= min_steps) S *= 2;
  return S;
}

static inline unsigned pyz_pad8(long long n, int P) { return (unsigned)(P > 1 ? (n + 7) / 8 * 8 : n); }

static inline bool pyz_fwd_takes_lds(const DenseArgs &g, int grid_batch, int P, int S) {
  const int lds_on = pyz_env_int("PYZ_FWD_LDS", 1);
  const bool lds_ok = g.K % 4 == 0 && g.N % 2 == 0 && g.lda % 4 == 0 && g.w_off % 2 == 0 && (P == 1 || g.theta_pstride % 2 == 0) &&
                      (P == 1 || g.in_pstride % 4 == 0) && (reinterpret_cast<uintptr_t>(g.theta) & 7) == 0 &&
                      (reinterpret_cast<uintptr_t>(g.in) & 15) == 0 &&
                      (!g.gather_out || (reinterpret_cast<uintptr_t>(g.gather_out) & 15) == 0);
  const int lds_max_rows = pyz_env_int("PYZ_FWD_LDS_MAXROWS", 2048);
  const int NT = g.N <= 64 ? 2 : (g.N <= 128 ? 4 : 7);
  const long long wg128 = (long long)((grid_batch + 127) / 128) * ((g.N + 32 * NT - 1) / (32 * NT)) * P;
  return S == 1 && !g.gate && lds_on && lds_ok && g.N >= 48 && grid_batch >= 128 && (grid_batch <= lds_max_rows || P >= 8) &&
         wg128 >= pyz_env_int("PYZ_FWD_LDS_MINWG", 256);
}

static inline void pyz_launch_fwd(const DenseArgs &g, int grid_batch, int P, hipStream_t st) {
  const long long tiles = (long long)((grid_batch + 31) / 32) * ((g.N + 31) / 32);
  const int S = pyz_pick_waves(tiles * P, (g.K + 1) / 2 + 1);
  if (pyz_fwd_takes_lds(g, grid_batch, P, S)) {
    const int NT = g.N <= 64 ? 2 : (g.N <= 128 ? 4 : 7);
    const long long tl = (long long)((grid_batch + 127) / 128) * ((g.N + 32 * NT - 1) / (32 * NT));
    const dim3 grid(pyz_pad8(tl, P), P), block(256);
    if (NT == 2) PYZ_LAUNCH(k_dense_fwd_lds<2>, grid, block, 0, st, g);
    else if (NT == 4) PYZ_LAUNCH(k_dense_fwd_lds<4>, grid, block, 0, st, g);
    else PYZ_LAUNCH(k_dense_fwd_lds<7>, grid, block, 0, st, g);
    return;
  }
  PYZ_LAUNCH(k_dense_fwd, dim3(pyz_pad8(tiles, P), P), dim3(64 * S), S > 1 ? S * 4096 : 0, st, g);
}

static inline void pyz_launch_bwd_data(const DenseArgs &g, int grid_batch, int P, hipStream_t st) {
  const long long tiles = (long long)((grid_batch + 31) / 32) * ((g.K + 31) / 32);
  const int S = pyz_pick_waves(tiles * P, (g.N + 1) / 2);
  PYZ_LAUNCH(k_dense_bwd_data, dim3(pyz_pad8(tiles, P), P), dim3(64 * S), S > 1 ? S * 4096 : 0, st, g);
}

static inline void pyz_launch_bwd_weight(const DenseArgs &g, int grid_batch, int P, hipStream_t st) {
  const long long tiles = (long long)((g.K + 1 + 31) / 32) * ((g.N + 31) / 32);
  const int S = pyz_pick_waves(tiles * P, (grid_batch + 1) / 2);
  PYZ_LAUNCH(k_dense_bwd_weight, dim3((unsigned)tiles, P), dim3(64 * S), S > 1 ? S * 4096 : 0, st, g);
}

static inline void pyz_launch_bwd_weight_sq(const DenseArgs &g, float *out2, int grid_batch, hipStream_t st) {
  const long long tiles = (long long)((g.K + 1 + 31) / 32) * ((g.N + 31) / 32);
  const int S = pyz_pick_waves(tiles, (grid_batch + 1) / 2);
  PYZ_LAUNCH(k_dense_bwd_weight_sq, dim3((unsigned)tiles), dim3(64 * S), S > 1 ? S * 4096 : 0, st, g, out2);
}
```

Measured before the change: 42620 grad-steps/s.

## Preload kernel arguments and specialize plain-path fronts for fwd, head and wgrad kernels

Enables kernarg preloading at compile time. The hot fields of the fwd, head_rows and wgrad_all kernels are passed as leading scalar arguments so they sit in preloaded SGPRs instead of being fetched from the argument struct. A packed flags word selects a specialized PLAIN path that skips gating, per-particle strides and the layer-table lookup. Integer tile division is replaced with a host-precomputed multiplicative inverse, and division by the wave count becomes a shift. The aim is to cut kernel prologue latency in a launch-bound small MLP step, at the cost of more code paths and new assumptions such as the power-of-two trap.

Result: faster. 44470 grad-steps/s (median of 6 runs) (+4.3%).

```diff
diff --git a/bayesian_inference_for_nn_amd/_build.py b/bayesian_inference_for_nn_amd/_build.py
--- a/bayesian_inference_for_nn_amd/_build.py
+++ b/bayesian_inference_for_nn_amd/_build.py
@@ -10,6 +10,7 @@
 CSRC = os.path.join(os.path.dirname(os.path.abspath(__file__)), "csrc")
 LIB = os.path.join(CSRC, "libpyz.so")
 SOURCES = ["pyz_api.hip"]
+PRELOAD = ["-mllvm", "-amdgpu-kernarg-preload-count=16"]
 
 
 class NoCompiler(RuntimeError):
@@ -41,7 +42,7 @@
                 return LIB
             tmp = LIB + f".tmp{os.getpid()}"
             cmd = [hipcc, "-O3", "-std=c++17", "--offload-arch=gfx950", "-fPIC", "-shared", "-Wall",
-                   "-Wno-unused-function", "-Wno-pass-failed"] + SOURCES + ["-o", tmp]
+                   "-Wno-unused-function", "-Wno-pass-failed"] + PRELOAD + SOURCES + ["-o", tmp]
             if verbose:
                 print(" ".join(cmd))
             res = subprocess.run(cmd, cwd=CSRC, capture_output=True, text=True)
diff --git a/bayesian_inference_for_nn_amd/csrc/pyz_api.hip b/bayesian_inference_for_nn_amd/csrc/pyz_api.hip
--- a/bayesian_inference_for_nn_amd/csrc/pyz_api.hip
+++ b/bayesian_inference_for_nn_amd/csrc/pyz_api.hip
@@ -330,18 +330,18 @@
     m->cur_nblk = g.nblk;
     static const int rw_rows = pyz_env_int("PYZ_HEAD_RW_ROWS", 32768);
     const int RW = (long long)P * grid_batch >= rw_rows ? 4 : 1;
-    const dim3 grid((unsigned)cdiv(cdiv(grid_batch, RW), 4), P), block(256);
+    const dim3 grid((unsigned)cdiv(cdiv(grid_batch, RW), 4), P);
     if (g.n_hparts > 0) {
-      if (NP == 4) PYZ_LAUNCH((k_head_rows<4, 4, 1, true>), grid, block, 0, st, g);
-      else if (NP == 8) PYZ_LAUNCH((k_head_rows<4, 8, 1, true>), grid, block, 0, st, g);
-      else if (NP == 12) PYZ_LAUNCH((k_head_rows<4, 12, 1, true>), grid, block, 0, st, g);
-      else PYZ_LAUNCH((k_head_rows<4, 16, 1, true>), grid, block, 0, st, g);
+      if (NP == 4) PYZ_LAUNCH_HEAD_ROWS((k_head_rows<4, 4, 1, true>), grid, st, g, P);
+      else if (NP == 8) PYZ_LAUNCH_HEAD_ROWS((k_head_rows<4, 8, 1, true>), grid, st, g, P);
+      else if (NP == 12) PYZ_LAUNCH_HEAD_ROWS((k_head_rows<4, 12, 1, true>), grid, st, g, P);
+      else PYZ_LAUNCH_HEAD_ROWS((k_head_rows<4, 16, 1, true>), grid, st, g, P);
       return;
     }
 #define PYZ_HEAD_ROWS_CASE(U, C)                                                               \
   if (UT == U && NP == C) {                                                                    \
-    if (RW == 4) PYZ_LAUNCH((k_head_rows<U, C, 4>), grid, block, 0, st, g);                     \
-    else PYZ_LAUNCH((k_head_rows<U, C, 1>), grid, block, 0, st, g);                            \
+    if (RW == 4) PYZ_LAUNCH_HEAD_ROWS((k_head_rows<U, C, 4>), grid, st, g, P);                  \
+    else PYZ_LAUNCH_HEAD_ROWS((k_head_rows<U, C, 1>), grid, st, g, P);                         \
     return;                                                                                    \
   }
     PYZ_HEAD_ROWS_CASE(1, 4) PYZ_HEAD_ROWS_CASE(1, 8) PYZ_HEAD_ROWS_CASE(1, 12) PYZ_HEAD_ROWS_CASE(1, 16)
@@ -411,6 +411,7 @@
     ly.w_off = m->w_off[l];
     ly.tile0 = tiles;
     a.tile0[l] = tiles;
+    ly.tn_mul = pyz_tilediv_mul((unsigned long long)((ly.K + 1 + 31) / 32) * ((ly.N + 31) / 32), (unsigned)((ly.N + 31) / 32));
     tiles += ((ly.K + 1 + 31) / 32) * ((ly.N + 31) / 32);
   }
   for (int l = m->L; l < PYZ_MAX_LAYERS; ++l) a.tile0[l] = INT_MAX;
@@ -432,13 +433,13 @@
   if (a.prep.src && P == 1) grid.x = (unsigned)(tiles + 1 + std::max(pyz_cu_count() - tiles - 1, 24));
   switch (S) {
     case 1:
-      if (a.mode == PYZ_UPD_NONE) PYZ_LAUNCH((k_wgrad_all<1, true>), grid, dim3(64), 0, st, a);
-      else PYZ_LAUNCH(k_wgrad_all<1>, grid, dim3(64), 0, st, a);
+      if (a.mode == PYZ_UPD_NONE) PYZ_LAUNCH((k_wgrad_all<1, true>), grid, dim3(64), 0, st, PYZ_WGRAD_ALL_ARGS(a, P));
+      else PYZ_LAUNCH(k_wgrad_all<1>, grid, dim3(64), 0, st, PYZ_WGRAD_ALL_ARGS(a, P));
       break;
-    case 2: PYZ_LAUNCH(k_wgrad_all<2>, grid, dim3(128), 2 * 4096, st, a); break;
-    case 4: PYZ_LAUNCH(k_wgrad_all<4>, grid, dim3(256), 4 * 4096, st, a); break;
-    case 8: PYZ_LAUNCH(k_wgrad_all<8>, grid, dim3(512), 8 * 4096, st, a); break;
-    default: PYZ_LAUNCH(k_wgrad_all<16>, grid, dim3(1024), 16 * 4096, st, a); break;
+    case 2: PYZ_LAUNCH(k_wgrad_all<2>, grid, dim3(128), 2 * 4096, st, PYZ_WGRAD_ALL_ARGS(a, P)); break;
+    case 4: PYZ_LAUNCH(k_wgrad_all<4>, grid, dim3(256), 4 * 4096, st, PYZ_WGRAD_ALL_ARGS(a, P)); break;
+    case 8: PYZ_LAUNCH(k_wgrad_all<8>, grid, dim3(512), 8 * 4096, st, PYZ_WGRAD_ALL_ARGS(a, P)); break;
+    default: PYZ_LAUNCH(k_wgrad_all<16>, grid, dim3(1024), 16 * 4096, st, PYZ_WGRAD_ALL_ARGS(a, P)); break;
   }
 }
 
diff --git a/bayesian_inference_for_nn_amd/csrc/pyz_fused.h b/bayesian_inference_for_nn_amd/csrc/pyz_fused.h
--- a/bayesian_inference_for_nn_amd/csrc/pyz_fused.h
+++ b/bayesian_inference_for_nn_amd/csrc/pyz_fused.h
@@ -438,25 +438,43 @@
   PYZ_STAMP(1, 5);
 }
 
-template <int UT, int NP, int RW = 1, bool HP = false>
-__global__ void __launch_bounds__(256) k_head_rows(HeadArgs g) {
-  PYZ_STAMP(1, 0);
+#define PYZ_HFRONT_PLAIN 1u
+#define PYZ_HFRONT_GATHER 2u
+#define PYZ_HFRONT_VEC 4u
+#define PYZ_HFRONT_WT 8u
+#define PYZ_HFRONT_LOSS(f) (int)(((f) >> 4) & 15u)
+#define PYZ_HFRONT_ACT_LAST(f) (int)(((f) >> 8) & 15u)
+#define PYZ_HFRONT_ACT_PREV(f) (int)(((f) >> 12) & 15u)
+static inline unsigned pyz_head_front_bits(const HeadArgs &g, int P) {
+  const bool plain = P == 1 && !g.gate && !g.init_on;
+  return (plain ? PYZ_HFRONT_PLAIN : 0u) | (g.gather_hin ? PYZ_HFRONT_GATHER : 0u) | (g.vec ? PYZ_HFRONT_VEC : 0u) |
+         (g.wt ? PYZ_HFRONT_WT : 0u) | ((unsigned)g.loss << 4) | ((unsigned)g.act_last << 8) | ((unsigned)g.act_prev << 12);
+}
+
+template <int UT, int NP, int RW, bool HP, bool PLAIN>
+__device__ __forceinline__ void pyz_head_rows_body(const HeadArgs &g, const PyzCtlHot &ctl_raw) {
   const int w = pyz_wave_id(), l = threadIdx.x & 63;
-  asm volatile("; arguments in one trip" ::"s"(g.hin), "s"(g.hin_pstride), "s"(g.theta), "s"(g.theta_pstride), "s"(g.w_off),
-               "s"(g.ctl), "s"(g.row_idx), "s"(g.gate), "s"(g.y), "s"(g.part), "s"(g.lda), "s"(g.K), "s"(g.N), "s"(g.loss),
-               "s"(g.gather_hin), "s"(g.gate_mod), "s"(g.init_on), "s"(g.nblk), "s"(g.act_last), "s"(g.act_prev), "s"(g.vec),
-               "s"(g.wt));
-  if (g.gate && g.gate->n % g.gate_mod == 0) return;
   StepCtl ctl;
-  if (g.init_on) {
-    asm volatile("; the step scalars by value" ::: "memory");
-    ctl = pyz_ctl_first(g.ctl, g.init, 1);
-  } else {
-    const PyzCtlHot c = pyz_ctl_arrived(pyz_ctl_request(g.ctl));
+  if (PLAIN) {
+    const PyzCtlHot c = pyz_ctl_arrived(ctl_raw);
     ctl.batch = c.batch;
     ctl.row_off = c.row_off;
-  }
-  const int batch = ctl.batch, p = blockIdx.y;
+  } else {
+    asm volatile("; arguments in one trip" ::"s"(g.hin_pstride), "s"(g.theta_pstride), "s"(g.gate), "s"(g.part), "s"(g.gate_mod),
+                 "s"(g.init_on), "s"(g.nblk));
+    PYZ_STAMP(1, 7);
+    if (g.gate && g.gate->n % g.gate_mod == 0) return;
+    if (g.init_on) {
+      asm volatile("; the step scalars by value" ::: "memory");
+      ctl = pyz_ctl_first(g.ctl, g.init, 1);
+    } else {
+      const PyzCtlHot c = pyz_ctl_arrived(ctl_raw);
+      ctl.batch = c.batch;
+      ctl.row_off = c.row_off;
+    }
+  }
+  PYZ_STAMP(1, 6);
+  const int batch = ctl.batch, p = PLAIN ? 0 : (int)blockIdx.y;
   const int m0 = (blockIdx.x * 4 + w) * RW;
   if (m0 >= batch) {
     if (l < RW && m0 + l < g.nblk) g.part[p * g.nblk + m0 + l] = 0.0;
@@ -478,6 +496,44 @@
     pyz_head_row<UT, NP, true>(g, batch, ctl.row_off, p, m, l, W);
   }
 }
+
+template <int UT, int NP, int RW = 1, bool HP = false>
+__global__ void __launch_bounds__(256) k_head_rows(const float *hin, const float *wb, const StepCtl *ctl, const int32_t *row_idx,
+                                                   const void *y, const int lda, const int K, const int N, const unsigned front,
+                                                   HeadArgs ga) {
+  PYZ_STAMP(1, 0);
+  const PyzCtlHot ctl_raw = pyz_ctl_request(ctl);
+  HeadArgs g = ga;
+  g.hin = hin;
+  g.theta = wb;
+  g.w_off = 0;
+  g.ctl = ctl;
+  g.row_idx = row_idx;
+  g.y = y;
+  g.lda = lda;
+  g.K = K;
+  g.N = N;
+  g.gather_hin = (front & PYZ_HFRONT_GATHER) ? 1 : 0;
+  g.vec = (front & PYZ_HFRONT_VEC) ? 1 : 0;
+  g.wt = (front & PYZ_HFRONT_WT) ? 1 : 0;
+  g.loss = PYZ_HFRONT_LOSS(front);
+  g.act_last = PYZ_HFRONT_ACT_LAST(front);
+  g.act_prev = PYZ_HFRONT_ACT_PREV(front);
+  if (__builtin_expect((front & PYZ_HFRONT_PLAIN) != 0u, 1)) {
+    PYZ_STAMP(1, 7);
+    g.hin_pstride = 0;
+    g.theta_pstride = 0;
+    g.gate = nullptr;
+    g.init_on = 0;
+    pyz_head_rows_body<UT, NP, RW, HP, true>(g, ctl_raw);
+  } else {
+    pyz_head_rows_body<UT, NP, RW, HP, false>(g, ctl_raw);
+  }
+}
+
+#define PYZ_LAUNCH_HEAD_ROWS(kern, grid, st, g, P)                                                                      \
+  PYZ_LAUNCH(kern, grid, dim3(256), 0, st, (g).hin, (g).theta + (g).w_off, (g).ctl, (g).row_idx, (g).y, (g).lda, (g).K, \
+             (g).N, pyz_head_front_bits(g, P), g)
 
 struct PrepArgs {
   const float *src;
@@ -598,6 +654,7 @@
   int lda, K, N;
   int tile0;
   int gather;
+  unsigned tn_mul;
 };
 
 #define PYZ_UPD_NONE 0
@@ -773,28 +830,74 @@
   }
 }
 
+#define PYZ_WFRONT_MODE 7u
+#define PYZ_WFRONT_FAST0 8u
+#define PYZ_WFRONT_GATHER0 16u
+struct PyzWgradFront {
+  int tiles;
+  unsigned front;
+  const float *in0, *delta0;
+  unsigned w_off0;
+  int lda0, K0, N0, tile0_1;
+  unsigned tn_mul0;
+};
+
 template <int S, bool PLAIN, int MODE>
-__device__ __forceinline__ void pyz_wgrad_tile(const WgradArgs &g, float *red) {
+__device__ __forceinline__ void pyz_wgrad_tile(const WgradArgs &g, float *red, const PyzWgradFront &f, PyzCtlHot ctl_raw) {
   constexpr int EPT = 16 / S;
   const int w = pyz_wave_id(), l = threadIdx.x & 63;
   const int r = l & 31, h = l >> 5;
-  const int tile = pyz_xcd_remap(blockIdx.x, g.tiles);
-  int li = 0;
-#pragma unroll
-  for (int j = 1; j < PYZ_MAX_LAYERS; ++j) li += tile >= g.tile0[j] ? 1 : 0;
-  li = __builtin_amdgcn_readfirstlane(li);
-  const WgradLayer &ly = g.lay[li];
-  const PyzCtlHot ctl_raw = pyz_ctl_request(g.ctl);
-  asm volatile("; the layer in one trip" ::"s"(ly.in), "s"(ly.in_pstride), "s"(ly.delta), "s"(ly.delta_pstride), "s"(ly.w_off),
-               "s"(ly.lda), "s"(ly.K), "s"(ly.N), "s"(ly.tile0), "s"(ly.gather));
+  const int tile = pyz_xcd_remap(blockIdx.x, f.tiles);
+  float *theta = g.theta, *mean = g.mean, *sq_mean = g.sq_mean;
+  const float *unit_noise = g.unit_noise;
+  const int32_t *row_idx = g.row_idx;
+  uint64_t seed = g.seed;
+  if constexpr (!PLAIN)
+    asm volatile("; arguments in one trip" : "+s"(theta), "+s"(mean), "+s"(sq_mean), "+s"(unit_noise), "+s"(row_idx), "+s"(seed));
+  PYZ_STAMP(2, 7);
+  const float *in_base, *delta_base;
+  long long w_off;
+  int lda, K, N, tile0, gather, p;
+  unsigned tn_mul;
+  if (!PLAIN && __builtin_expect((f.front & PYZ_WFRONT_FAST0) && tile < f.tile0_1, 1)) {
+    in_base = f.in0;
+    delta_base = f.delta0;
+    w_off = (long long)f.w_off0;
+    lda = f.lda0;
+    K = f.K0;
+    N = f.N0;
+    tile0 = 0;
+    gather = (f.front & PYZ_WFRONT_GATHER0) ? 1 : 0;
+    tn_mul = f.tn_mul0;
+    p = 0;
+  } else {
+    asm volatile("; the layer table is needed here" ::: "memory");
+    int li = 0;
+#pragma unroll
+    for (int j = 1; j < PYZ_MAX_LAYERS; ++j) li += tile >= g.tile0[j] ? 1 : 0;
+    li = __builtin_amdgcn_readfirstlane(li);
+    const WgradLayer &ly = g.lay[li];
+    if constexpr (PLAIN) ctl_raw = pyz_ctl_request(g.ctl);
+    asm volatile("; the layer in one trip" ::"s"(ly.in), "s"(ly.in_pstride), "s"(ly.delta), "s"(ly.delta_pstride), "s"(ly.w_off),
+                 "s"(ly.lda), "s"(ly.K), "s"(ly.N), "s"(ly.tile0), "s"(ly.gather), "s"(ly.tn_mul));
+    p = blockIdx.y;
+    in_base = ly.in + p * ly.in_pstride;
+    delta_base = ly.delta + p * ly.delta_pstride;
+    w_off = ly.w_off;
+    lda = ly.lda;
+    K = ly.K;
+    N = ly.N;
+    tile0 = ly.tile0;
+    gather = ly.gather;
+    tn_mul = ly.tn_mul;
+  }
   const PyzCtlHot ctl = pyz_ctl_arrived(ctl_raw);
+  PYZ_STAMP(2, 6);
   const int batch = ctl.batch;
-  const int K = ly.K, N = ly.N;
   const int tiles_n = (N + 31) >> 5;
-  const int t = tile - ly.tile0;
-  const int i0 = (t / tiles_n) * 32, n0 = (t % tiles_n) * 32;
-  const int p = blockIdx.y;
-  const long long w_off = ly.w_off;
+  const int t = tile - tile0;
+  const int tq = PLAIN ? t / tiles_n : (int)pyz_tilediv((unsigned)t, (unsigned)tiles_n, tn_mul);
+  const int i0 = tq * 32, n0 = (PLAIN ? t % tiles_n : t - tq * tiles_n) * 32;
   constexpr int mode = PLAIN ? PYZ_UPD_NONE : MODE;
   const long long nstep = ctl.n;
   const float lr = ctl.lr;
@@ -822,42 +925,41 @@
       ee[q] = w_off + (long long)min(ii, K) * N + min(nn, N - 1);
       if (PLAIN) continue;
       th0[q] = mu0[q] = sq0[q] = zz[q] = zg[q] = 0.0f;
-      if (mode != PYZ_UPD_NONE) th0[q] = g.theta[ee[q]];
+      if (mode != PYZ_UPD_NONE) th0[q] = theta[ee[q]];
       if (mode == PYZ_UPD_SGLD || mode == PYZ_UPD_BBB || mode == PYZ_UPD_SWAG) {
-        mu0[q] = g.mean[ee[q]];
-        sq0[q] = g.sq_mean[ee[q]];
-        if (g.unit_noise && mode != PYZ_UPD_SWAG) zz[q] = g.unit_noise[ee[q]];
-      }
-    }
-    if (!PLAIN && (mode == PYZ_UPD_SGLD || mode == PYZ_UPD_BBB) && !g.unit_noise) {
+        mu0[q] = mean[ee[q]];
+        sq0[q] = sq_mean[ee[q]];
+        if (unit_noise && mode != PYZ_UPD_SWAG) zz[q] = unit_noise[ee[q]];
+      }
+    }
+    if (!PLAIN && (mode == PYZ_UPD_SGLD || mode == PYZ_UPD_BBB) && !unit_noise) {
 #pragma unroll
       for (int q = 0; q < EPT; ++q) {
-        zg[q] = mode == PYZ_UPD_SGLD ? pyz_normal1(g.seed, PYZ_STREAM_SGLD, (uint32_t)nstep, (uint64_t)ee[q])
-                                     : pyz_normal1(g.seed, PYZ_STREAM_BBB, g.bbb_chained ? (uint32_t)nstep : g.bbb_step, (uint64_t)ee[q]);
+        zg[q] = mode == PYZ_UPD_SGLD ? pyz_normal1(seed, PYZ_STREAM_SGLD, (uint32_t)nstep, (uint64_t)ee[q])
+                                     : pyz_normal1(seed, PYZ_STREAM_BBB, g.bbb_chained ? (uint32_t)nstep : g.bbb_step, (uint64_t)ee[q]);
       }
     }
     if (!PLAIN && fuse_next) {
 #pragma unroll
-      for (int q = 0; q < EPT; ++q) zn[q] = pyz_normal1(g.seed, PYZ_STREAM_BBB, (uint32_t)(nstep + 1), (uint64_t)ee[q]);
+      for (int q = 0; q < EPT; ++q) zn[q] = pyz_normal1(seed, PYZ_STREAM_BBB, (uint32_t)(nstep + 1), (uint64_t)ee[q]);
     }
   };
 
   const int i = i0 + r, n = min(n0 + r, N - 1);
   const int ic = min(i, K - 1);
   const bool is_w = i < K, is_b = i == K;
-  const float *ap = ly.in + p * ly.in_pstride + ic;
-  const float *dp = ly.delta + p * ly.delta_pstride + n;
-  const int32_t *idx = (ly.gather && g.row_idx) ? g.row_idx + ctl.row_off : nullptr;
+  const float *ap = in_base + ic;
+  const float *dp = delta_base + n;
+  const int32_t *idx = (gather && row_idx) ? row_idx + ctl.row_off : nullptr;
   f32x16 acc = {0};
   const int steps = (batch + 1) >> 1;
-  int s = (steps * w) / S;
-  const int se = (steps * (w + 1)) / S;
+  int s = (int)((unsigned)(steps * w) / (unsigned)S);
+  const int se = (int)((unsigned)(steps * (w + 1)) / (unsigned)S);
   PYZ_STAMP(2, 1);
   if (idx) {
     prefetch();
     for (int s0 = s; s0 < se; s0 += 32) {
       const int idxv = idx[min(2 * s0 + l, batch - 1)];
-      const int lda = ly.lda;
       pyz_steps1_all(
           s0, min(s0 + 32, se), acc,
           [&](int st, float &a, float &d) {
@@ -873,8 +975,7 @@
           });
     }
   } else {
-    pyz_wgrad_accumulate(acc, ly.in + p * ly.in_pstride, ic, ly.delta + p * ly.delta_pstride, n, ly.lda, N, batch, s, se, h,
-                         is_w, is_b, prefetch);
+    pyz_wgrad_accumulate(acc, in_base, ic, delta_base, n, lda, N, batch, s, se, h, is_w, is_b, prefetch);
   }
   PYZ_STAMP(2, 2);
   float gv[EPT];
@@ -946,15 +1047,15 @@
 }
 
 template <int S, bool PLAIN = false>
-__global__ void __launch_bounds__(64 * S) k_wgrad_all(WgradArgs g) {
+__global__ void __launch_bounds__(64 * S) k_wgrad_all(const int tiles, const unsigned front, const StepCtl *ctl, const float *in0,
+                                                      const float *delta0, const unsigned w_off0, const int lda0, const int K0,
+                                                      const int N0, const int tile0_1, const unsigned tn_mul0, WgradArgs g) {
   extern __shared__ float red[];
   PYZ_STAMP(2, 0);
+  PyzCtlHot ctl_raw{};
+  if constexpr (!PLAIN) ctl_raw = pyz_ctl_request(ctl);
   const int w = pyz_wave_id(), l = threadIdx.x & 63;
-  asm volatile("; arguments in one trip" ::"s"(g.tiles), "s"(g.mode), "s"(g.ctl), "s"(g.row_idx), "s"(g.tile0[1]),
-               "s"(g.tile0[2]), "s"(g.tile0[3]), "s"(g.tile0[4]), "s"(g.tile0[5]), "s"(g.tile0[6]), "s"(g.tile0[7]),
-               "s"(g.tile0[8]), "s"(g.tile0[9]), "s"(g.tile0[10]), "s"(g.tile0[11]), "s"(g.tile0[12]), "s"(g.tile0[13]),
-               "s"(g.tile0[14]), "s"(g.tile0[15]));
-  if (blockIdx.x >= (unsigned)g.tiles) {
+  if (__builtin_expect(blockIdx.x >= (unsigned)tiles, 0)) {
     if (blockIdx.x == (unsigned)g.tiles && blockIdx.y == 0 && w == 0) pyz_step_duties(g, l);
     if (blockIdx.x == (unsigned)g.tiles && w == 0 && g.ploss) {
       const double tot = pyz_sum_partials(g.part + (long long)blockIdx.y * g.nblk, g.nblk);
@@ -972,18 +1073,28 @@
     }
     return;
   }
+  const PyzWgradFront f{tiles, front, in0, delta0, w_off0, lda0, K0, N0, tile0_1, tn_mul0};
   if constexpr (PLAIN) {
-    pyz_wgrad_tile<S, true, PYZ_UPD_NONE>(g, red);
+    pyz_wgrad_tile<S, true, PYZ_UPD_NONE>(g, red, f, ctl_raw);
   } else {
-    switch (g.mode) {
-      case PYZ_UPD_SGLD: pyz_wgrad_tile<S, false, PYZ_UPD_SGLD>(g, red); break;
-      case PYZ_UPD_SGD: pyz_wgrad_tile<S, false, PYZ_UPD_SGD>(g, red); break;
-      case PYZ_UPD_SWAG: pyz_wgrad_tile<S, false, PYZ_UPD_SWAG>(g, red); break;
-      case PYZ_UPD_BBB: pyz_wgrad_tile<S, false, PYZ_UPD_BBB>(g, red); break;
-      default: pyz_wgrad_tile<S, false, PYZ_UPD_NONE>(g, red); break;
-    }
-  }
-}
+    switch ((int)(front & PYZ_WFRONT_MODE)) {
+      case PYZ_UPD_SGLD: pyz_wgrad_tile<S, false, PYZ_UPD_SGLD>(g, red, f, ctl_raw); break;
+      case PYZ_UPD_SGD: pyz_wgrad_tile<S, false, PYZ_UPD_SGD>(g, red, f, ctl_raw); break;
+      case PYZ_UPD_SWAG: pyz_wgrad_tile<S, false, PYZ_UPD_SWAG>(g, red, f, ctl_raw); break;
+      case PYZ_UPD_BBB: pyz_wgrad_tile<S, false, PYZ_UPD_BBB>(g, red, f, ctl_raw); break;
+      default: pyz_wgrad_tile<S, false, PYZ_UPD_NONE>(g, red, f, ctl_raw); break;
+    }
+  }
+}
+
+static inline unsigned pyz_wgrad_front_bits(const WgradArgs &a, int P) {
+  const WgradLayer &l0 = a.lay[0];
+  const bool fast0 = P == 1 && l0.w_off >= 0 && l0.w_off <= 0xFFFFFFFFll && l0.in_pstride == 0 && l0.tile0 == 0;
+  return (unsigned)a.mode | (fast0 ? PYZ_WFRONT_FAST0 : 0u) | ((l0.gather && a.row_idx) ? PYZ_WFRONT_GATHER0 : 0u);
+}
+#define PYZ_WGRAD_ALL_ARGS(a, P)                                                                                          \
+  (a).tiles, pyz_wgrad_front_bits(a, P), (a).ctl, (a).lay[0].in, (a).lay[0].delta, (unsigned)(a).lay[0].w_off, (a).lay[0].lda, \
+      (a).lay[0].K, (a).lay[0].N, (a).tile0[1], (a).lay[0].tn_mul, a
 
 template <class H>
 __device__ __forceinline__ void pyz_wgrad_accumulate_sq(f32x16 &acc, f32x16 &acc2, const float fb, const float *abase,
diff --git a/bayesian_inference_for_nn_amd/csrc/pyz_gemm.h b/bayesian_inference_for_nn_amd/csrc/pyz_gemm.h
--- a/bayesian_inference_for_nn_amd/csrc/pyz_gemm.h
+++ b/bayesian_inference_for_nn_amd/csrc/pyz_gemm.h
@@ -3,6 +3,7 @@
 #include <cstdlib>
 
 #include "pyz_common.h"
+#include "pyz_tilediv.h"
 
 struct DenseArgs {
   const float *in;
@@ -100,8 +101,8 @@
 }
 
 template <class F>
-__device__ __forceinline__ void pyz_tile_epilogue(const f32x16 &acc, float *red, F store) {
-  const int S = blockDim.x >> 6, w = pyz_wave_id(), l = threadIdx.x & 63;
+__device__ __forceinline__ void pyz_tile_epilogue(const f32x16 &acc, float *red, F store, const int S) {
+  const int w = pyz_wave_id(), l = threadIdx.x & 63;
   const int r = l & 31, h = l >> 5;
   if (S == 1) {
 #pragma unroll
@@ -120,6 +121,10 @@
     default: __builtin_trap();
   }
 }
+template <class F>
+__device__ __forceinline__ void pyz_tile_epilogue(const f32x16 &acc, float *red, F store) {
+  pyz_tile_epilogue(acc, red, store, (int)(blockDim.x >> 6));
+}
 
 struct PyzNoFix {
   __device__ __forceinline__ void operator()(int, float &, float &) const {}
@@ -230,15 +235,17 @@
 __device__ __forceinline__ void pyz_fwd_accumulate(f32x16 &acc, const float *ap, const float *wl, const int n, const int K,
                                                    const int N, const int vec, const int w, const int S, const int h,
                                                    float *gp = nullptr, const int copy_mod = 1, const int copy_rem = 0,
-                                                   H hook = H()) {
-  const __amdgpu_buffer_rsrc_t rw =
-      __builtin_amdgcn_make_buffer_rsrc(const_cast<float *>(wl), 0, (int)((unsigned)(K + 1) * (unsigned)N * 4u), 0x00020000);
+                                                   H hook = H(), const unsigned wb_bytes = 0u) {
+  const __amdgpu_buffer_rsrc_t rw = __builtin_amdgcn_make_buffer_rsrc(
+      const_cast<float *>(wl), 0, (int)(wb_bytes ? wb_bytes : (unsigned)(K + 1) * (unsigned)N * 4u), 0x00020000);
   const unsigned n4 = 4u * (unsigned)n, N4 = 4u * (unsigned)N;
   const float bias = pyz_buf_load(rw, n4, (unsigned)K * N4);
+  if ((S & (S - 1)) != 0) __builtin_trap();
+  const int lgS = __builtin_ctz((unsigned)S);
   const int c8 = vec ? (K >> 3) : 0;
   const unsigned v0 = (4u * h) * N4 + n4, v1 = v0 + N4, v2 = v1 + N4, v3 = v2 + N4;
   pyz_steps4_all(
-      0, (c8 - w + S - 1) / S, acc,
+      0, (c8 - w + S - 1) >> lgS, acc,
       [&](int u, float4 &a4, float4 &b4) {
         const int c = PYZ_HOT(w + S * u, K);
         a4 = *reinterpret_cast<const float4 *>(ap + 8 * c + 4 * h);
@@ -261,7 +268,7 @@
   const int t0 = 8 * c8, steps = (K - t0 + 1) >> 1;
   const unsigned vt = (unsigned)h * N4 + n4;
   pyz_steps1_all(
-      0, (steps - w + S - 1) / S, acc,
+      0, (steps - w + S - 1) >> lgS, acc,
       [&](int u, float &a, float &b) {
         const int kb = t0 + 2 * (w + S * u);
         const int kk = kb + h;
@@ -280,51 +287,79 @@
   }
 }
 
-__global__ void k_dense_fwd(DenseArgs g) {
-  extern __shared__ float red[];
-  PYZ_STAMP(0, 0);
-  const int S = blockDim.x >> 6, w = pyz_wave_id(), l = threadIdx.x & 63;
+#define PYZ_FRONT_VEC 1u
+#define PYZ_FRONT_PLAIN 2u
+#define PYZ_FRONT_WT 4u
+#define PYZ_FRONT_LGS(f) (((f) >> 4) & 7u)
+#define PYZ_FRONT_ACT(f) (int)(((f) >> 8) & 15u)
+static inline unsigned pyz_front_bits(const DenseArgs &g, int P, int S) {
+  int lg = 0;
+  while ((1 << lg) < S) ++lg;
+  const bool plain = P == 1 && g.rows_cap > 0 && !g.gate && !g.row_idx && !g.gather_out && !g.init_on;
+  return (g.vec ? PYZ_FRONT_VEC : 0u) | (plain ? PYZ_FRONT_PLAIN : 0u) | (g.wt ? PYZ_FRONT_WT : 0u) | ((unsigned)lg << 4) |
+         ((unsigned)g.act << 8);
+}
+
+template <bool PLAIN>
+__device__ __forceinline__ void pyz_dense_fwd_tile(const float *in, const float *wb, const StepCtl *ctlp, const int lda, const int K,
+                                                   const int N, const int rows_cap, const unsigned grid_x, const unsigned front,
+                                                   const unsigned tn_mul, const unsigned wb_bytes, const DenseArgs &g, float *red) {
+  const int S = 1 << PYZ_FRONT_LGS(front), w = pyz_wave_id(), l = threadIdx.x & 63;
   const int r = l & 31, h = l >> 5;
-  const int tiles_n = (g.N + 31) >> 5;
-  asm volatile("; arguments in one trip" ::"s"(g.in), "s"(g.in_pstride), "s"(g.theta), "s"(g.theta_pstride), "s"(g.w_off),
-               "s"(g.lda), "s"(g.K), "s"(g.N), "s"(g.vec), "s"(g.rows_cap), "s"(g.gate_mod), "s"(g.out), "s"(g.out_pstride),
-               "s"(g.ctl), "s"(g.row_idx), "s"(g.gather_out), "s"(g.gate), "s"(g.act), "s"(g.wt), "s"((int)gridDim.x),
-               "s"((int)blockDim.x));
-  if (g.gate && g.gate->n % g.gate_mod == 0) return;
-  const int tile = pyz_xcd_remap(blockIdx.x, gridDim.x);
-  const int m0 = (tile / tiles_n) * 32, n0 = (tile % tiles_n) * 32;
-  int cap = g.rows_cap;
+  const int tiles_n = (N + 31) >> 5;
+  if (!PLAIN) {
+    asm volatile("; arguments in one trip" ::"s"(g.in_pstride), "s"(g.theta_pstride), "s"(g.gate_mod), "s"(g.out), "s"(g.out_pstride),
+                 "s"(g.row_idx), "s"(g.gather_out), "s"(g.gate));
+    PYZ_STAMP(0, 7);
+    if (g.gate && g.gate->n % g.gate_mod == 0) return;
+  }
+  const int tile = pyz_xcd_remap(blockIdx.x, (int)grid_x);
+  const int tq = (int)pyz_tilediv((unsigned)tile, (unsigned)tiles_n, tn_mul), tr = tile - tq * tiles_n;
+  const int m0 = tq * 32, n0 = tr * 32;
+  int cap = rows_cap;
   long long row_off = 0;
-  if (cap <= 0) {
+  if (!PLAIN && cap <= 0) {
     asm volatile("; the step scalars are needed here" ::: "memory");
-    const StepCtl ctl = pyz_ctl_first(g.ctl, g.init, g.init_on);
+    const StepCtl ctl = pyz_ctl_first(ctlp, g.init, g.init_on);
     cap = __builtin_amdgcn_readfirstlane(ctl.batch);
     row_off = ctl.row_off;
   }
   if (m0 >= cap) return;
-  const int p = blockIdx.y;
-  const int K = g.K, N = g.N;
+  const int p = PLAIN ? 0 : (int)blockIdx.y;
   const int m = min(m0 + r, cap - 1), n = min(n0 + r, N - 1);
   long long row = m;
-  if (g.row_idx) row = g.row_idx[row_off + m];
-  const float *ap = g.in + p * g.in_pstride + row * g.lda;
-  const float *wl = g.theta + p * g.theta_pstride + g.w_off;
+  if (!PLAIN && g.row_idx) row = g.row_idx[row_off + m];
+  const float *ap = PLAIN ? in + row * lda : in + p * g.in_pstride + row * lda;
+  const float *wl = PLAIN ? wb : wb + p * g.theta_pstride;
   f32x16 acc = {0};
   PYZ_STAMP(0, 1);
-  float *gp = (g.gather_out && p == 0) ? g.gather_out + (long long)m * K : nullptr;
+  float *gp = (!PLAIN && g.gather_out && p == 0) ? g.gather_out + (long long)m * K : nullptr;
   int batch = 0;
-  const int32_t *ctl_batch = &g.ctl->batch;
-  pyz_fwd_accumulate(acc, ap, wl, n, K, N, g.vec, w, S, h, gp, tiles_n, tile % tiles_n,
-                     [&]() { batch = __hip_atomic_load(ctl_batch, __ATOMIC_RELAXED, __HIP_MEMORY_SCOPE_AGENT); });
-  batch = g.rows_cap > 0 ? __builtin_amdgcn_readfirstlane(batch) : cap;
+  const int32_t *ctl_batch = &ctlp->batch;
+  pyz_fwd_accumulate(acc, ap, wl, n, K, N, (int)(front & PYZ_FRONT_VEC), w, S, h, gp, tiles_n, tr,
+                     [&]() { batch = __hip_atomic_load(ctl_batch, __ATOMIC_RELAXED, __HIP_MEMORY_SCOPE_AGENT); }, wb_bytes);
+  batch = rows_cap > 0 ? __builtin_amdgcn_readfirstlane(batch) : cap;
   PYZ_STAMP(0, 2);
-  float *op = g.out + p * g.out_pstride;
-  const int act = g.act, wt = g.wt;
+  float *op = PLAIN ? g.out : g.out + p * g.out_pstride;
+  const int act = PYZ_FRONT_ACT(front), wt = (front & PYZ_FRONT_WT) ? 1 : 0;
   pyz_tile_epilogue(acc, red, [&](int ro, int co, float v) {
     const int mm = m0 + ro, nn = n0 + co;
     if (mm < batch && nn < N) pyz_st(op + (long long)mm * N + nn, pyz_act(v, act), wt);
-  });
+  }, S);
   PYZ_STAMP(0, 3);
+}
+
+__global__ void k_dense_fwd(const float *in, const float *wb, const StepCtl *ctl, const int lda, const int K, const int N,
+                            const int rows_cap, const unsigned grid_x, const unsigned front, const unsigned tn_mul,
+                            const unsigned wb_bytes, DenseArgs g) {
+  extern __shared__ float red[];
+  PYZ_STAMP(0, 0);
+  if (__builtin_expect((front & PYZ_FRONT_PLAIN) != 0u, 1)) {
+    PYZ_STAMP(0, 7);
+    pyz_dense_fwd_tile<true>(in, wb, ctl, lda, K, N, rows_cap, grid_x, front, tn_mul, wb_bytes, g, red);
+  } else {
+    pyz_dense_fwd_tile<false>(in, wb, ctl, lda, K, N, rows_cap, grid_x, front, tn_mul, wb_bytes, g, red);
+  }
 }
 
 template <int NT>
@@ -674,7 +709,10 @@
     else PYZ_LAUNCH(k_dense_fwd_lds<7>, grid, block, 0, st, g);
     return;
   }
-  PYZ_LAUNCH(k_dense_fwd, dim3(pyz_pad8(tiles, P), P), dim3(64 * S), S > 1 ? S * 4096 : 0, st, g);
+  const unsigned grid_x = pyz_pad8(tiles, P), tiles_n = (unsigned)((g.N + 31) / 32);
+  PYZ_LAUNCH(k_dense_fwd, dim3(pyz_pad8(tiles, P), P), dim3(64 * S), S > 1 ? S * 4096 : 0, st, g.in, g.theta + g.w_off, g.ctl,
+             g.lda, g.K, g.N, g.rows_cap, grid_x, pyz_front_bits(g, P, S), pyz_tilediv_mul(grid_x, tiles_n),
+             (unsigned)(g.K + 1) * (unsigned)g.N * 4u, g);
 }
 
 static inline void pyz_launch_bwd_data(const DenseArgs &g, int grid_batch, int P, hipStream_t st) {
diff --git a/bayesian_inference_for_nn_amd/csrc/pyz_tilediv.h b/bayesian_inference_for_nn_amd/csrc/pyz_tilediv.h
--- /dev/null
+++ b/bayesian_inference_for_nn_amd/csrc/pyz_tilediv.h
@@ -0,0 +1,20 @@
+#pragma once
+
+#if defined(__HIPCC__) || defined(__CUDACC__)
+#define PYZ_HD __host__ __device__
+#else
+#define PYZ_HD
+#endif
+
+#define PYZ_TILEDIV_MAX_TILES (1u << 16)
+#define PYZ_TILEDIV_MAX_D (1u << 11)
+
+PYZ_HD inline unsigned pyz_tilediv_mul(const unsigned long long tiles, const unsigned d) {
+  if (d < 2u || d > PYZ_TILEDIV_MAX_D || tiles > PYZ_TILEDIV_MAX_TILES) return 0u;
+  return (unsigned)((0x100000000ull + d - 1u) / d);
+}
+
+PYZ_HD inline unsigned pyz_tilediv(const unsigned tile, const unsigned d, const unsigned mul) {
+  if (__builtin_expect(mul != 0u, 1)) return (unsigned)(((unsigned long long)tile * mul) >> 32);
+  return d == 1u ? tile : tile / d;
+}
```
